# ubisoft/ubisoft-laforge-msmd

Hardware: AMD Instinct MI355X
Metric: FLAME frames/sec on 4s@16kHz clips (whole job; MSMD.forward motion-coefficient frames) (higher is better)
Workload: dtype bf16; 1 GPU; configs[1]: MSMD.forward, batch=32 x 4 s clips per GPU, wav2vec2-base encoder + 8-layer motion decoder, eval-mode, synthetic closed-form weights; batch_per_gpu=32, frames_per_clip=100, parallelism=dp1 (independent clips, no collective), launch=one hipGraph replay per step (the batch sits in the captured input buffers)

## Files before the change

### include/msmd_hip.h

```cpp
#ifndef MSMD_HIP_H
#define MSMD_HIP_H

#include <stdint.h>

#ifdef __cplusplus
extern "C" {
#endif

#define MSMD_F32 0
#define MSMD_BF16 1
#define MSMD_F16 2
#define MSMD_F16X2 3

#define MSMD_ACT_NONE 0
#define MSMD_ACT_GELU 1
#define MSMD_ACT_ELU 2

typedef void* msmd_stream_t;

int msmd_abi_version(void);
#define MSMD_GEMM_VARIANT(v) ((v) << 8)
#define MSMD_GEMM_WRITE_THROUGH (1 << 16)
#define MSMD_GEMM_PAIRED_STORES (1 << 17)
#define MSMD_GEMM_STAGGER (1 << 18)
#define MSMD_GEMM_ONE_TILE_PER_WORKGROUP (1 << 19)
#define MSMD_GEMM_NO_256_TILE (1 << 20)
#define MSMD_GEMM_W_BELOW_32 (1 << 21)

int msmd_spin_us(float us, long* ticks_out, msmd_stream_t stream);

int msmd_gemm(const void* A, const void* W, const float* bias, const void* residual, void* C,
              int M, int N, int K, int in_dtype, int out_dtype,
              long lda, int rows_per_batch, long a_batch_stride, long ldw, long ldc, long ldr, int act,
              int batch, long strideA, long strideW, long strideC, long strideBias, long strideR,
              msmd_stream_t stream);

int msmd_gemm_ln(const void* A, const void* W, const float* bias, const void* residual, void* C, int M, int N, int K,
                 int in_dtype, int out_dtype, long lda, long ldw, long ldc, long ldr, int act, const float* a_stats,
                 const float* w_colsum, const float* r_stats, const float* r_gamma, const float* r_beta,
                 float* stats_out, int slab_in, int slab_out, float eps, msmd_stream_t stream);

int msmd_gemm_ex(const void* A, const void* W, const float* bias, const void* residual, void* C, int M, int N, int K,
                 int in_dtype, int out_dtype, long lda, int rows_per_batch, long a_batch_stride, long ldw, long ldc,
                 long ldr, int act, int batch, long strideA, long strideW, long strideC, long strideBias, long strideR,
                 void* z_out, float p_drop, const unsigned long* rng_state, unsigned int site, msmd_stream_t stream);

int msmd_gemm_route(const void* A, const void* W, const float* bias, const void* residual, void* C, int M, int N, int K,
                    int in_dtype, int out_dtype, long lda, int rows_per_batch, long a_batch_stride, long ldw, long ldc,
                    long ldr, int act, int batch, long strideA, long strideW, long strideC, long strideBias, long strideR,
                    void* z_out, float p_drop, const unsigned long* rng_state, unsigned int site, msmd_stream_t stream);
int msmd_gemm_ln_route(const void* A, const void* W, const float* bias, const void* residual, void* C, int M, int N, int K,
                       int in_dtype, int out_dtype, long lda, long ldw, long ldc, long ldr, int act, const float* a_stats,
                       const float* w_colsum, const float* r_stats, const float* r_gamma, const float* r_beta,
                       float* stats_out, int slab_in, int slab_out, float eps, msmd_stream_t stream);

int msmd_gemm_actbwd(const void* A, const void* W, const void* Z, void* C, int M, int N, int K, int in_dtype, int out_dtype,
                     long lda, long ldw, int act, float p_drop, const unsigned long* rng_state, unsigned int site,
                     msmd_stream_t stream);

int msmd_gemm_batched2(const void* A, const void* W, void* C, int M, int N, int K, int in_dtype, int out_dtype,
                       long lda, long ldw, long ldc, int batch_outer, long strideA_o, long strideW_o, long strideC_o,
                       int batch_inner, long strideA_i, long strideW_i, long strideC_i, msmd_stream_t stream);

int msmd_gemm_tn(const void* A, const void* B, float* C, float* colsum, int M, int N, int K, long lda, long ldb,
                 long ldc, int batch, long strideA, long strideB, long strideC, int b_rows_per_window,
                 long b_window_stride, int accumulate, void* ws, long ws_bytes, msmd_stream_t stream);
long msmd_gemm_tn_workspace(int M, int N, int K, int batch);

int msmd_layernorm(const void* x, const void* residual, const float* gamma, const float* beta,
                   const float* post_add, void* y, int rows, int cols, float eps, int act,
                   int in_dtype, int out_dtype, msmd_stream_t stream);
int msmd_layernorm_pre(const void* x, const float* pre_gamma, const float* pre_beta, const void* residual,
                       const float* gamma, const float* beta, void* y, int rows, int cols, float eps, int dtype,
                       msmd_stream_t stream);

int msmd_layernorm_f16x2(const float* x, const float* residual, const float* gamma, const float* beta,
                         const float* post_add, float* y, void* y_split, int rows, int cols, float eps, int act,
                         msmd_stream_t stream);

int msmd_split_f16x2(const float* x, void* y, long rows, int cols, long ldx, int cols_out, msmd_stream_t stream);
int msmd_unsplit_f16x2(const void* x, float* y, long rows, int cols, int cols_in, long ldy, msmd_stream_t stream);

int msmd_attention_prefetch(const void* Q, const void* K, const void* V, void* O, int B, int H, int Tq, int Tk,
                            long q_bstride, long q_tstride, long k_bstride, long k_tstride, long v_bstride,
                            long v_tstride, long o_bstride, long o_tstride, float scale, const uint8_t* mask, int dtype,
                            const void* const* prefetch_ptrs, const long* prefetch_bytes, int n_prefetch,
                            msmd_stream_t stream);
int msmd_attention(const void* Q, const void* K, const void* V, void* O, int B, int H, int Tq, int Tk,
                   long q_bstride, long q_tstride, long k_bstride, long k_tstride, long v_bstride,
                   long v_tstride, long o_bstride, long o_tstride, float scale, const uint8_t* mask,
                   int dtype, msmd_stream_t stream);

int msmd_attention_f16x2(const void* Q, const void* K, const void* V, void* O, int B, int H, int Tq, int Tk,
                         long q_bstride, long q_tstride, long k_bstride, long k_tstride, long v_bstride,
                         long v_tstride, long o_bstride, long o_tstride, float scale, const uint8_t* mask,
                         int out_dtype, msmd_stream_t stream);


int msmd_person_query_attention(const void* x, long x_seq_stride, const void* Wq, const float* bq, const void* K,
                                const void* V, long kv_bstride, long kv_tstride, void* out, int N, int H, int Tk, int d,
                                float scale, int dtype, msmd_stream_t stream);
int msmd_person_query_attention_ln(const void* x, long x_seq_stride, const void* Wq, const float* bq,
                                   const float* wq_colsum, float ln_eps, const void* K, const void* V, long kv_bstride,
                                   long kv_tstride, void* out, int N, int H, int Tk, int d, float scale, int dtype,
                                   msmd_stream_t stream);

int msmd_attention_dropout(const void* Q, const void* K, const void* V, void* O, int B, int H, int Tq, int Tk,
                           long q_bstride, long q_tstride, long k_bstride, long k_tstride, long v_bstride,
                           long v_tstride, long o_bstride, long o_tstride, float scale, const uint8_t* mask,
                           float p_drop, const unsigned long* rng_state, unsigned int site, int dtype,
                           msmd_stream_t stream);
int msmd_attention_dropout_prefetch(const void* Q, const void* K, const void* V, void* O, int B, int H, int Tq, int Tk,
                                    long q_bstride, long q_tstride, long k_bstride, long k_tstride, long v_bstride,
                                    long v_tstride, long o_bstride, long o_tstride, float scale, const uint8_t* mask,
                                    float p_drop, const unsigned long* rng_state, unsigned int site, int dtype,
                                    const void* const* prefetch_ptrs, const long* prefetch_bytes, int n_prefetch,
                                    msmd_stream_t stream);

int msmd_dropout(const void* x, const void* residual, void* y, long n, float p, const unsigned long* rng_state,
                 unsigned int site, int dtype, msmd_stream_t stream);

int msmd_attention_bwd(const void* Q, const void* K, const void* V, const void* dO, void* dQ, void* dK, void* dV,
                       int B, int H, int Tq, int Tk, long q_bstride, long q_tstride, long k_bstride,
                       long k_tstride, long v_bstride, long v_tstride, long do_bstride, long do_tstride,
                       long dq_bstride, long dq_tstride, long dk_bstride, long dk_tstride, long dv_bstride,
                       long dv_tstride, float scale, const uint8_t* mask, float p_drop,
                       const unsigned long* rng_state, unsigned int site, msmd_stream_t stream);

int msmd_pad_audio(const float* audio, float* out, int B, int L, int reflect_len, int replicate_len,
                   msmd_stream_t stream);

#define MSMD_CONV0_SPLITS 16
int msmd_conv0_stats(const float* audio, const float* w0, float* stats, float* ws, int B, int L, int reflect_len,
                     int replicate_len, int C, float eps, msmd_stream_t stream);

int msmd_conv0_gn_gelu(const float* audio, const float* w0, const float* stats, const float* gamma,
                       const float* beta, void* out, int B, int L, int reflect_len, int replicate_len,
                       int C, int out_dtype, msmd_stream_t stream);

int msmd_conv0_ln_gelu(const float* audio, const float* w0, const float* bias, const float* gamma, const float* beta,
                       void* out, int B, int L, int reflect_len, int replicate_len, int C, float eps, int out_dtype,
                       msmd_stream_t stream);

int msmd_interp_linear(const void* x, void* y, int B, int T_in, int T_crop, int T_out, int C, int dtype,
                       msmd_stream_t stream);

int msmd_group_pad(const void* x, void* y, int B, int T, int G, int Cg, int Cg_out, int pad, int dtype, int out_dtype,
                   msmd_stream_t stream);

int msmd_pos_conv(const void* x, const void* w, const float* bias, void* y, int B, int T, int G, int Cg, int kpos,
                  int dtype, msmd_stream_t stream);

int msmd_denoiser_pack_input(const float* motion, const float* eps, const float* c0, const float* c1,
                             const float* prev_motion, const float* indicator, void* feats, int N, int L,
                             int Lp, int dm, int Kpad, int motion_batch, int out_dtype, msmd_stream_t stream);

int msmd_denoiser_pack_input_guided(const float* motion, const float* eps, const float* c0, const float* c1,
                                    const float* prev_motion, const float* indicator, const unsigned char* guide_mask,
                                    const float* guide_values, void* feats, int N, int L, int Lp, int dm, int Kpad,
                                    int motion_batch, int out_dtype, msmd_stream_t stream);

int msmd_add_pe_token(void* x, const float* pe, const void* tok0, const void* row0_add, int N, int T, int d,
                      int dtype, msmd_stream_t stream);

int msmd_heads_static_mix(const void* dec, long ld_dec, const void* stat, float* out, int N, int L, int dm,
                          int nb, int stat_batch, int use_head_alpha, int dtype, msmd_stream_t stream);

int msmd_cfg_ddpm_step(float* x, const float* res, const float* z, const float* scales, int n_entries,
                       int B, int L, int Lp, int dm, int mode, int target, float c0, float c1, float sigma,
                       msmd_stream_t stream);

int msmd_sampler_step_select(const void* emb_all, const float* coef_table, int* t_dev, void* emb_row,
                             float* coefs, int d, int dtype, msmd_stream_t stream);
int msmd_cfg_ddpm_step_dev(float* x, const float* res, const float* z, const float* scales, const float* coefs,
                           int n_entries, int B, int L, int Lp, int dm, int mode, int target, msmd_stream_t stream);

int msmd_cfg_solver_step(float* x, const float* res, const float* z, const float* scales, float* d_prev,
                         int n_entries, int B, int L, int Lp, int dm, int mode, float p0, float p1, float ax,
                         float ath, float b1, float sigma, msmd_stream_t stream);
int msmd_cfg_solver_step_dev(float* x, const float* res, const float* z, const float* scales, float* d_prev,
                             const float* coefs, int n_entries, int B, int L, int Lp, int dm, int mode,
                             msmd_stream_t stream);
int msmd_sampler_solver_select(const void* emb_tab, const float* coef_tab, int* i_dev, void* emb_row,
                               float* coefs, int d, int dtype, msmd_stream_t stream);

int msmd_cfg_streams_step(float* x, const float* res, const void* dec, long ld_dec, const void* stat, const float* z,
                          const float* scales, float* d_prev, float* cum_static, float* theta_dyn, float* theta_alpha,
                          int slot, int n_slots, int n_entries, int B, int L, int Lp, int dm, int nb, int stat_batch,
                          int use_head_alpha, int mode, int dtype, float p0, float p1, float ax, float ath, float b1,
                          float sigma, msmd_stream_t stream);
int msmd_cfg_streams_step_dev(float* x, const float* res, const void* dec, long ld_dec, const void* stat, const float* z,
                              const float* scales, float* d_prev, float* cum_static, float* theta_dyn,
                              float* theta_alpha, const float* coefs, const int* step_dev, int n_slots, int n_entries,
                              int B, int L, int Lp, int dm, int nb, int stat_batch, int use_head_alpha, int mode,
                              int dtype, msmd_stream_t stream);

int msmd_lbs_prepare(const float* betas, const float* pose, const float* JS, const int* parents,
                     float* coef, void* coef_hl, float* A, float* joints, void* at_tiles, int B, int NB, int J, int Kp,
                     int pose_is_matrix, msmd_stream_t stream);
int msmd_flame_prepare(const float* shape, const float* expr, const float* pose6, const float* eye, const float* JS,
                       const int* parents, float* coef, float* A, float* joints, void* skin_tiles, int B, int NS, int NE,
                       int ignore_global_rot, int* shape_varies, float* v_template_folded, const float* dirs,
                       const float* v_template, int Vp, msmd_stream_t stream);
int msmd_lbs_skin(const float* coef, const float* A, const float* v_template, const float* dirs,
                  const float* lbs_weights, float* verts, int B, int J, int V, int Vp, int Kp,
                  msmd_stream_t stream);
int msmd_lbs_skin_bf16x3(const void* coef_hl, const float* A, const float* v_template, const void* dirs_hl,
                         const float* lbs_weights, float* verts, int B, int J, int V, int Vp, int Kp,
                         msmd_stream_t stream);

int msmd_lbs_skin_v2(const void* skin_tiles, const float* v_template, const void* dirs_hl, const float* lbs_weights,
                     float* verts, int B, int J, int V, int Vp, int Kp, const int* shape_varies,
                     const float* v_template_folded, msmd_stream_t stream);

int msmd_lbs_skin_v2_f16(const void* skin_tiles, const float* v_template, const void* dirs, const float* lbs_weights,
                         void* verts16, int B, int J, int V, int V_ld, int Vp, int Kp, const int* shape_varies,
                         const float* v_template_folded, int single_plane, msmd_stream_t stream);
int msmd_lbs_tiles_f16(const void* skin_tiles, void* tiles16, int B, msmd_stream_t stream);

int msmd_lbs_skin_v2_train(const void* skin_tiles, const float* v_template, const void* dirs_hl,
                           const float* lbs_weights, float* verts, float* v_posed, int B, int J, int V, int Vp, int Kp,
                           msmd_stream_t stream);
int msmd_lbs_pack(const float* coef, const float* A, void* coef_hl, void* skin_tiles, int B, int Kp, msmd_stream_t stream);
int msmd_lbs_skin_bwd(const float* grad_verts, const float* v_posed, const float* A, const float* lbs_weights,
                      float* dp_planes, float* dA, int B, int J, int V, int Vp, msmd_stream_t stream);

int msmd_landmarks(const float* verts, const int* faces, const int* lmk_faces_idx, long idx_bstride,
                   const float* bary, long bary_bstride, float* out, int B, int V, int L, msmd_stream_t stream);

int msmd_landmarks_bwd(const float* grad_lmk, const int* faces, const int* lmk_faces_idx, long idx_bstride,
                       const float* bary, long bary_bstride, float* grad_verts, int B, int V, int L, int accumulate,
                       msmd_stream_t stream);

int msmd_dynamic_lmk_row(const float* full_pose, const int* neck_chain, int n_chain, int* row, int B, int J,
                         int pose_is_matrix, msmd_stream_t stream);

int msmd_batch_rodrigues(const float* rot_vecs, float* R, int N, msmd_stream_t stream);
int msmd_batch_rodrigues_bwd(const float* rot_vecs, const float* grad_R, float* grad_rot_vecs, int N, msmd_stream_t stream);

#define MSMD_ROT_QUAT_TO_MAT 0
#define MSMD_ROT_MAT_TO_QUAT 1
#define MSMD_ROT_AA_TO_QUAT 2
#define MSMD_ROT_QUAT_TO_AA 3
#define MSMD_ROT_AA_TO_MAT 4
#define MSMD_ROT_MAT_TO_AA 5
#define MSMD_ROT_6D_TO_MAT 6
#define MSMD_ROT_MAT_TO_6D 7
#define MSMD_ROT_AA_TO_6D 8
#define MSMD_ROT_EULER_TO_MAT 9
#define MSMD_ROT_MAT_TO_EULER 10
#define MSMD_ROT_QUAT_STANDARDIZE 11
#define MSMD_ROT_QUAT_INVERT 12
#define MSMD_ROT_QUAT_RAW_MUL 13
#define MSMD_ROT_QUAT_MUL 14
#define MSMD_ROT_QUAT_APPLY 15
int msmd_rotation_convert(int op, const float* in, const float* in2, float* out, long n, int conv,
                          msmd_stream_t stream);
int msmd_rotation_convert_bwd(int op, const float* in, const float* in2, const float* grad_out, float* grad_in,
                              float* grad_in2, long n, int conv, msmd_stream_t stream);

int msmd_masked_seq_loss(const float* gt, const float* pred, const int* end_idx, float* out, double* acc_ws,
                         int N, int T, int C, int c_lo, int c_hi, int order, int prefix, int criterion, int mode,
                         float scale, msmd_stream_t stream);
int msmd_masked_seq_loss_bwd(const float* gt, const float* pred, const int* end_idx, const double* acc_ws,
                             const float* upstream, float* grad_pred, int N, int T, int C, int c_lo, int c_hi, int order,
                             int prefix, int criterion, int mode, float scale, msmd_stream_t stream);
int msmd_kl_loss(const float* mu, const float* logvar, float* out, double* acc_ws, long n, msmd_stream_t stream);
int msmd_truncate_rows(float* x, const int* end_idx, int N, int L, int inner, int unit, int replicate,
                       msmd_stream_t stream);
int msmd_adam_step(float* param, const float* grad, float* exp_avg, float* exp_avg_sq, long n, float lr,
                   float beta1, float beta2, float eps, int step, float grad_scale, msmd_stream_t stream);

int msmd_comm_version(void);
int msmd_comm_unique_id(void* id_out_128_bytes);
int msmd_comm_init(void** comm_out, int world, int rank, const void* id_128_bytes);
int msmd_comm_destroy(void* comm);
int msmd_allreduce_bucket(void* comm, void* buf, long n, int dtype, msmd_stream_t stream);

int msmd_transpose(const void* x, void* y, int rows, int cols, long ldx, long ldy, int batch, long stride_x,
                   long stride_y, int batch_inner, long stride_x_i, long stride_y_i, int dtype, msmd_stream_t stream);
long msmd_colsum_workspace(long rows, int cols);
int msmd_colsum(const void* x, float* out, long rows, int cols, long ld, int accumulate, int dtype, void* ws, long ws_bytes,
                msmd_stream_t stream);
int msmd_act_fwd(const void* z, void* y, long n, int act, int dtype, msmd_stream_t stream);
int msmd_act_bwd(const void* dy, const void* z, void* dz, long n, int act, int dtype, msmd_stream_t stream);
int msmd_act_bwd_dropout(const void* dy, const void* z, void* dz, long n, int act, float p,
                         const unsigned long* rng_state, unsigned int site, int dtype, msmd_stream_t stream);
int msmd_layernorm_bwd(const void* dy, const void* x, const float* gamma, void* dx, float* dgamma, float* dbeta,
                       int rows, int cols, float eps, int dtype, void* ws, long ws_bytes, msmd_stream_t stream);
long msmd_layernorm_bwd_workspace(int rows, int cols);
int msmd_layernorm_bwd_dropout(const void* dy, const void* x, const float* gamma, void* dx, void* dx_drop, float* dgamma,
                               float* dbeta, int rows, int cols, float eps, float p_drop, const unsigned long* rng_state,
                               unsigned int site, int dtype, void* ws, long ws_bytes, msmd_stream_t stream);
int msmd_softmax_rows(void* s, const uint8_t* mask, long rows, int cols, int ld, int Tq, float scale, int dtype,
                      msmd_stream_t stream);
int msmd_softmax_bwd_rows(const void* P, void* dP, long rows, int cols, int ld, float scale, int dtype,
                          msmd_stream_t stream);

int msmd_unfold_t(const void* xp, void* out, int B, int T, int Tp, int G, int Cg, int Kk, long ld_out, int dtype,
                  msmd_stream_t stream);

int msmd_cast(const void* x, void* y, long n, int in_dtype, int out_dtype, msmd_stream_t stream);
int msmd_pad_cols(const void* x, void* y, long rows, int cols_in, int cols_out, int in_dtype, int out_dtype,
                  msmd_stream_t stream);
int msmd_mean_time(const void* x, float* y, int B, int T, int C, int dtype, msmd_stream_t stream);

int msmd_dynamic_threshold(float* res, int N, int T_all, int L, int C, float ratio, float dt_min, float dt_max,
                           msmd_stream_t stream);

int msmd_cast_transpose_multi(const float* base, const long* meta, int n_weights, long total_tiles, void* cast_arena,
                              void* transposed_arena, msmd_stream_t stream);

int msmd_batch_windows(const float* audio_flat, const float* coef_flat, const long* desc, const float* clip_stats,
                       const float* coef_mean, const float* coef_std, float* out_audio, float* out_motion, int B, int L,
                       int C, int n_audio, double audio_unit, msmd_stream_t stream);

int msmd_render_vertices(const float* verts, const int* faces, const int* csr_offsets, const int* csr_faces,
                         const float* view, const float* t_center, const float* rot, float* screen, float* normals,
                         int B, int V, int F, float focal, int H, int W, msmd_stream_t stream);
int msmd_render_raster(const float* screen, const float* normals, const int* faces, const float* shade,
                       const float* lights, int n_lights, void* rgba, float* depth, int* face_id, int B, int V, int F,
                       int H, int W, float near, float far, unsigned background, msmd_stream_t stream);

long msmd_texture_texels(int Ht, int Wt);
int msmd_texture_mips(const void* img, int Ht, int Wt, int channels, float* pyramid, msmd_stream_t stream);
int msmd_render_shade_textured(const float* screen, const float* normals, const int* faces, const float* vt, const int* ft,
                               const float* pyramid, int Ht, int Wt, const float* shade, const float* lights,
                               int n_lights, const int* face_id, void* rgba, float* uvl, int B, int V, int F, int Nt,
                               int H, int W, float near, msmd_stream_t stream);

#define MSMD_TEX_PLANAR_F32 0
#define MSMD_TEX_IMAGE_U8 1
int msmd_flametex_forward(const float* mean, const float* basis, const float* code, void* out, int out_format, int n_copies,
                          int Hs, int Ws, int Hd, int Wd, int n_tex, msmd_stream_t stream);
long msmd_flametex_backward_workspace(int Hd, int Wd, int n_tex);
int msmd_flametex_backward(const float* basis, const float* grad_out, int n_copies, float* grad_code, float* workspace,
                           int Hs, int Ws, int Hd, int Wd, int n_tex, msmd_stream_t stream);

#define MSMD_AUDIO_RUN 256
int msmd_audio_resample(const void* pcm, long pcm_elems, int is_int16, const long* desc, int n_clips, long max_out_len,
                        int L, int M, int taps, const float* bank, float* out, long out_elems, double* partials,
                        msmd_stream_t stream);
int msmd_audio_znorm(float* out, long out_elems, const long* desc, int n_clips, long max_out_len, const double* partials,
                     double* stats, msmd_stream_t stream);

#define MSMD_JPEG_RESTART_INTERVAL 32
#define MSMD_JPEG_MAX_SIDE 16384
int msmd_jpeg_intervals(int H, int W);
int msmd_jpeg_coefficients(const void* frames, long frame_stride, long row_stride, int pixel_stride, int B, int H, int W,
                           int quality, short* coef, msmd_stream_t stream);
int msmd_jpeg_measure(const short* coef, int B, int H, int W, int header_len, int* interval_len, long* interval_rel,
                      long* frame_size, long* offsets, msmd_stream_t stream);
int msmd_jpeg_write(const short* coef, int B, int H, int W, const void* header, int header_len, const long* interval_rel,
                    const long* offsets, void* out, long out_bytes, msmd_stream_t stream);

#ifdef __cplusplus
}
// ... 3 lines not shown
```

### ubisoft-laforge-msmd_amd/csrc/gemm.hip

```cpp
#include "common.h"
#include <atomic>
#include <utility>

struct GemmArgs {
  const void* A; const void* W; const float* bias; const void* R; void* C;
  int M, N, K;
  long lda; int rows_per_batch; long a_batch_stride; long ldw, ldc, ldr;
  int act; int vec_ok; float inv_rpb;
  long strideA, strideW, strideC, strideBias, strideR;
  int mt, nt;
  int batch_inner; long strideA2, strideW2, strideC2;
  void* Z; float p_drop; const unsigned long* rng; unsigned site;
  int xn;
  int flags;
  const float* a_stats = nullptr; int a_nt = 0; const float* w_colsum = nullptr;
  const float* r_stats = nullptr; int r_nt = 0; const float* r_gamma = nullptr; const float* r_beta = nullptr;
  float* stats_out = nullptr; float ln_eps = 1e-5f;
  int stagger_ticks = 0;
};

enum : int {
  GF_WRITE_THROUGH = 1, GF_PAIRED_STORES = 2, GF_STAGGER = 4,
  GF_ACT_BWD = 8,
  GF_ONE_TILE = 16, GF_NO_256 = 32,
  GF_W_BELOW_32 = 64,
};
struct GemmActWord { int act, hint, flags; };
static constexpr GemmActWord gemm_unpack_act(int act) {
  return {act & 0xff, (act >> 8) & 0xff, ((act >> 16) & 7) | (((act >> 19) & 7) << 4)};
}
static_assert(gemm_unpack_act(MSMD_GEMM_WRITE_THROUGH).flags == GF_WRITE_THROUGH && gemm_unpack_act(MSMD_GEMM_PAIRED_STORES).flags == GF_PAIRED_STORES &&
              gemm_unpack_act(MSMD_GEMM_STAGGER).flags == GF_STAGGER && gemm_unpack_act(MSMD_GEMM_ONE_TILE_PER_WORKGROUP).flags == GF_ONE_TILE &&
              gemm_unpack_act(MSMD_GEMM_NO_256_TILE).flags == GF_NO_256 && gemm_unpack_act(MSMD_GEMM_W_BELOW_32).flags == GF_W_BELOW_32 && gemm_unpack_act(~0).flags == (0x7f & ~GF_ACT_BWD),
              "internal flag bits follow include/msmd_hip.h; no bit of `act` sets the internal one");
enum : int {
  GV_GENERIC = 0,
  GV_SPLIT_128 = 1, GV_SPLIT_64 = 5,
  GV_64_DEEP = 9, GV_64 = 12,
  GV_256x64 = 14,
  GV_192 = 15,
  GV_128 = 17,
  GV_128_AB = 13, GV_128_ONE_AB = 66,
  GV_256 = 80,
};

enum GemmEpi : int { EPI_ALL = 0, EPI_PLAIN = 1, EPI_LN_OPERAND = 2, EPI_LN_RESIDUAL = 3 };
constexpr int ACT_RUNTIME = -1;
constexpr int epia(GemmEpi e, int act) { return e + 10 * (1 + act); }
constexpr GemmEpi epia_family(int code) { return (GemmEpi)(code % 10); }
constexpr int epia_act(int code) { return code / 10 - 1; }

template <typename T> struct Mfma;
template <> struct Mfma<bf16_t> {
  static __device__ __forceinline__ void run(const u32x4& a, const u32x4& b, f32x4& acc) {
    acc = __builtin_amdgcn_mfma_f32_16x16x32_bf16(__builtin_bit_cast(bf16x8, a), __builtin_bit_cast(bf16x8, b),
                                                  acc, 0, 0, 0);
  }
};
template <> struct Mfma<f16_t> {
  static __device__ __forceinline__ void run(const u32x4& a, const u32x4& b, f32x4& acc) {
    acc = __builtin_amdgcn_mfma_f32_16x16x32_f16(__builtin_bit_cast(f16x8, a), __builtin_bit_cast(f16x8, b), acc, 0, 0, 0);
  }
};
template <> struct Mfma<float> {
  static __device__ __forceinline__ void run(const u32x4& a, const u32x4& b, f32x4& acc) {
#pragma unroll
    for (int e = 0; e < 4; ++e)
      acc = __builtin_amdgcn_mfma_f32_16x16x4f32(__uint_as_float(a[e]), __uint_as_float(b[e]), acc, 0, 0, 0);
  }
};

__device__ __forceinline__ int lds_off(int row, int chunk) { return row * 128 + ((chunk ^ ((row >> 1) & 7)) << 4); }

__device__ __forceinline__ long a_row_offset(const GemmArgs& p, int m) {
  if (p.rows_per_batch >= p.M) return (long)m * p.lda;
  int q = (int)((float)m * p.inv_rpb);
  int r = m - q * p.rows_per_batch;
  if (r < 0) { q -= 1; r += p.rows_per_batch; }
  if (r >= p.rows_per_batch) { q += 1; r -= p.rows_per_batch; }
  return (long)q * p.a_batch_stride + (long)r * p.lda;
}

template <typename TO> __device__ __forceinline__ float act_out(float x, int act) {
  if (act == MSMD_ACT_GELU) return sizeof(TO) == 2 ? gelu_poly16(x) : gelu_erf(x);
  if (act == MSMD_ACT_ELU) return elu1(x);
  return x;
}
template <typename TO, int ACT> __device__ __forceinline__ float act_out_c(float x, int act) {
  if constexpr (ACT == MSMD_ACT_GELU) return sizeof(TO) == 2 ? gelu_poly16(x) : gelu_erf(x);
  else if constexpr (ACT == MSMD_ACT_ELU) return elu1(x);
  else if constexpr (ACT == MSMD_ACT_NONE) return x;
  else return act_out<TO>(x, act);
}

__device__ __forceinline__ void store16_wt(void* p, const u32x4 v) {
  asm volatile("global_store_dwordx4 %0, %1, off sc1\n\ts_nop 1" ::"v"(p), "v"(v) : "memory");
}
__device__ __forceinline__ void store8_wt(void* p, const u32x2 v) {
  asm volatile("global_store_dwordx2 %0, %1, off sc1\n\ts_nop 1" ::"v"(p), "v"(v) : "memory");
}
template <typename TO> __device__ __forceinline__ void store4_out(TO* p, const float* v, bool wt) {
  if constexpr (sizeof(TO) == 4) {
    const f32x4 o = f32x4{v[0], v[1], v[2], v[3]};
    if (wt) store16_wt(p, __builtin_bit_cast(u32x4, o));
    else *(f32x4*)p = o;
  } else {
    const typename Vec4T<TO>::type o = pack4<TO>(v[0], v[1], v[2], v[3]);
    if (wt) store8_wt(p, __builtin_bit_cast(u32x2, o));
    else *(typename Vec4T<TO>::type*)p = o;
  }
}

template <typename TO, int FM, int FN, bool AB, bool LEAN, int ACT>
__device__ __forceinline__ void gemm_epilogue_interior(const GemmArgs& p, const f32x4 (&acc)[FN][FM], int z, int m_base,
                                                         int n_base, int fr, int fq) {
  TO* __restrict__ C = (TO*)p.C + (z / p.batch_inner) * p.strideC + (z % p.batch_inner) * p.strideC2 +
                       (long)(m_base + fr) * p.ldc + n_base + fq * 4;
  const TO* __restrict__ R = p.R ? (const TO*)p.R + z * p.strideR + (long)(m_base + fr) * p.ldr + n_base + fq * 4 : nullptr;
  const float* __restrict__ bias = p.bias ? p.bias + z * p.strideBias + n_base + fq * 4 : nullptr;
  const bool wt = p.flags & GF_WRITE_THROUGH;
  f32x4 bv[FN];
#pragma unroll
  for (int i = 0; i < FN; ++i) bv[i] = bias ? *(const f32x4*)(bias + i * 16) : f32x4{0.f, 0.f, 0.f, 0.f};
  typedef typename Vec4T<TO>::type V4;
  constexpr int RJ = sizeof(TO) == 2 ? FM : 1;
  V4 rr[RJ][FN];
  auto load_residual = [&](int j0) {
    if (R) {
#pragma unroll
      for (int j = 0; j < RJ; ++j)
#pragma unroll
        for (int i = 0; i < FN; ++i) rr[j][i] = *(const V4*)(R + (long)(j0 + j) * 16 * p.ldr + i * 16);
    }
  };
  if constexpr (RJ == FM) load_residual(0);
  auto finish = [&](int i, int j, float (&v)[4]) {
    TO* crow = C + (long)j * 16 * p.ldc;
#pragma unroll
    for (int e = 0; e < 4; ++e) v[e] = acc[i][j][e] + bv[i][e];
    if (AB && (p.flags & GF_ACT_BWD)) {
      const V4 z4 = *(const V4*)((const TO*)p.Z + (crow + i * 16 - (TO*)p.C));
#pragma unroll
      for (int e = 0; e < 4; ++e) v[e] *= act_grad_fast((float)z4[e], ACT >= 0 ? ACT : p.act);
    } else {
      if (!LEAN && p.Z) store4_out<TO>((TO*)p.Z + (crow + i * 16 - (TO*)p.C), v, wt);
#pragma unroll
      for (int e = 0; e < 4; ++e) v[e] = act_out_c<TO, ACT>(v[e], p.act);
    }
    if (!LEAN && p.p_drop > 0.f) {
      const long idx = (long)(m_base + j * 16 + fr) * p.N + (n_base + i * 16 + fq * 4);
      const Philox4 rb = dropout_bits(p.rng, p.site, (unsigned long)(idx >> 2));
      const unsigned thr = dropout_threshold(p.p_drop);
      const float c = 1.0f / (1.0f - p.p_drop);
      v[0] = rb.x >= thr ? v[0] * c : 0.f;
      v[1] = rb.y >= thr ? v[1] * c : 0.f;
      v[2] = rb.z >= thr ? v[2] * c : 0.f;
      v[3] = rb.w >= thr ? v[3] * c : 0.f;
    }
    if (R) {
#pragma unroll
      for (int e = 0; e < 4; ++e) v[e] += (float)rr[j % RJ][i][e];
    }
  };
  if constexpr (sizeof(TO) == 2 && FM % 2 == 0) {
    if (p.flags & GF_PAIRED_STORES) {
      const bool odd = fq & 1;
#pragma unroll
      for (int jp = 0; jp < FM / 2; ++jp) {
#pragma unroll
        for (int i = 0; i < FN; ++i) {
          float v0[4], v1[4];
          finish(i, 2 * jp, v0);
          finish(i, 2 * jp + 1, v1);
          const u32x2 a = __builtin_bit_cast(u32x2, pack4<TO>(v0[0], v0[1], v0[2], v0[3]));
          const u32x2 b = __builtin_bit_cast(u32x2, pack4<TO>(v1[0], v1[1], v1[2], v1[3]));
          const u32x2 send = odd ? a : b;
          u32x2 recv;
          recv[0] = __shfl_xor(send[0], 16, 64);
          recv[1] = __shfl_xor(send[1], 16, 64);
          const u32x4 o = odd ? u32x4{recv[0], recv[1], b[0], b[1]} : u32x4{a[0], a[1], recv[0], recv[1]};
          TO* dst = C + (long)(2 * jp + (odd ? 1 : 0)) * 16 * p.ldc + i * 16 - (odd ? 4 : 0);
          if (wt) store16_wt(dst, o);
          else *(u32x4*)dst = o;
        }
      }
      return;
    }
  }
#pragma unroll
  for (int j = 0; j < FM; ++j) {
    if constexpr (RJ != FM) load_residual(j);
#pragma unroll
    for (int i = 0; i < FN; ++i) {
      float v[4];
      finish(i, j, v);
      store4_out<TO>(C + (long)j * 16 * p.ldc + i * 16, v, wt);
    }
  }
}

template <typename TO, int FM, int FN, bool AB = false, bool LEAN = false, int ACT = -1>
__device__ __forceinline__ void gemm_epilogue(const GemmArgs& p, const f32x4 (&acc)[FN][FM], int z, int m_base,
                                              int n_base, int fr, int fq) {
  if (p.vec_ok && m_base + FM * 16 <= p.M && n_base + FN * 16 <= p.N) {
    gemm_epilogue_interior<TO, FM, FN, AB, LEAN, ACT>(p, acc, z, m_base, n_base, fr, fq);
    return;
  }
  TO* __restrict__ C = (TO*)p.C + (z / p.batch_inner) * p.strideC + (z % p.batch_inner) * p.strideC2;
  const TO* __restrict__ R = p.R ? (const TO*)p.R + z * p.strideR : nullptr;
  const float* __restrict__ bias = p.bias ? p.bias + z * p.strideBias : nullptr;
#pragma unroll
  for (int i = 0; i < FN; ++i) {
    const int n = n_base + i * 16 + fq * 4;
    if (n >= p.N) continue;
    float bv[4] = {0.f, 0.f, 0.f, 0.f};
    if (bias) {
#pragma unroll
      for (int e = 0; e < 4; ++e) bv[e] = (n + e < p.N) ? bias[n + e] : 0.f;
    }
#pragma unroll
    for (int j = 0; j < FM; ++j) {
      const int m = m_base + j * 16 + fr;
      if (m >= p.M) continue;
      float v[4];
#pragma unroll
      for (int e = 0; e < 4; ++e) v[e] = acc[i][j][e] + bv[e];
      TO* cp = C + (long)m * p.ldc + n;
      if (AB && (p.flags & GF_ACT_BWD)) {
        const TO* zp = (const TO*)p.Z + (cp - (TO*)p.C);
#pragma unroll
        for (int e = 0; e < 4; ++e)
          if (n + e < p.N) v[e] *= act_grad_fast((float)zp[e], ACT >= 0 ? ACT : p.act);
      } else {
        if (!LEAN && p.Z) {
          TO* zp = (TO*)p.Z + (cp - (TO*)p.C);
#pragma unroll
          for (int e = 0; e < 4; ++e)
            if (n + e < p.N) zp[e] = (TO)v[e];
        }
#pragma unroll
        for (int e = 0; e < 4; ++e) v[e] = act_out_c<TO, ACT>(v[e], p.act);
      }
      if (!LEAN && p.p_drop > 0.f) {
        const Philox4 rb = dropout_bits(p.rng, p.site, (unsigned long)(((long)m * p.N + n) >> 2));
        const unsigned thr = dropout_threshold(p.p_drop);
        const float c = 1.0f / (1.0f - p.p_drop);
        v[0] = rb.x >= thr ? v[0] * c : 0.f;
        v[1] = rb.y >= thr ? v[1] * c : 0.f;
        v[2] = rb.z >= thr ? v[2] * c : 0.f;
        v[3] = rb.w >= thr ? v[3] * c : 0.f;
      }
      if (p.vec_ok && n + 3 < p.N) {
        if (R) {
          const TO* rp = R + (long)m * p.ldr + n;
          if constexpr (sizeof(TO) == 4) {
            const f32x4 r = *(const f32x4*)rp;
#pragma unroll
            for (int e = 0; e < 4; ++e) v[e] += r[e];
          } else {
            const typename Vec4T<TO>::type r = *(const typename Vec4T<TO>::type*)rp;
#pragma unroll
            for (int e = 0; e < 4; ++e) v[e] += (float)r[e];
          }
        }
        store4_out<TO>(cp, v, p.flags & GF_WRITE_THROUGH);
      } else {
#pragma unroll
        for (int e = 0; e < 4; ++e) {
          if (n + e < p.N) {
            float o = v[e];
            if (R) o += to_f32(R[(long)m * p.ldr + n + e]);
            cp[e] = from_f32<TO>(o);
          }
        }
      }
    }
  }
}

template <int FM>
__device__ __forceinline__ void ln_issue(const float* stats, int nt, int M, int m_base, int fr, int fq, f32x2 (&raw)[FM][4]) {
#pragma unroll
  for (int j = 0; j < FM; ++j) {
    const f32x2* sp = (const f32x2*)stats + min(m_base + j * 16 + fr, M - 1);
#pragma unroll
    for (int q = 0; q < 4; ++q) raw[j][q] = fq + 4 * q < nt ? sp[(long)(fq + 4 * q) * M] : f32x2{0.f, 0.f};
  }
}

template <int FM>
__device__ __forceinline__ void ln_finish(const float* stats, int nt, int M, int m_base, int fr, int fq, const f32x2 (&raw)[FM][4],
                                          float inv_cols, float eps, float (&mu)[FM], float (&rs)[FM]) {
#pragma unroll
  for (int j = 0; j < FM; ++j) {
    float S = (raw[j][0][0] + raw[j][1][0]) + (raw[j][2][0] + raw[j][3][0]);
    float Q = (raw[j][0][1] + raw[j][1][1]) + (raw[j][2][1] + raw[j][3][1]);
    if (nt > 16) {
      const f32x2* sp = (const f32x2*)stats + min(m_base + j * 16 + fr, M - 1);
      for (int t = 16 + fq; t < nt; t += 4) { const f32x2 w = sp[(long)t * M]; S += w[0]; Q += w[1]; }
    }
    S += __shfl_xor(S, 16, 64); S += __shfl_xor(S, 32, 64);
    Q += __shfl_xor(Q, 16, 64); Q += __shfl_xor(Q, 32, 64);
    mu[j] = S * inv_cols;
    rs[j] = rsqrtf(fmaxf(Q * inv_cols - mu[j] * mu[j], 0.f) + eps);
  }
}

template <typename TO, int FM, int FN, int MODE, int ACT = -1>
__device__ __forceinline__ void gemm_epilogue_ln(const GemmArgs& p, const f32x4 (&acc)[FN][FM], int m_base, int n_base,
                                                 int fr, int fq, const f32x2 (&raw)[FM][4]) {
  static_assert((FN == 4 || FN == 2) && (FM >= 2 && FM <= 4), "one wave = one statistics slab of 16 FN columns, 2 to 4 fragment rows");
  constexpr int SLAB = FN * 16;
  constexpr int IB = FM == 3 ? 2 : FN;
  typedef typename Vec4T<TO>::type V4;
  const int n = n_base + fq * 4;
  float mu[FM], rs[FM];
#pragma unroll
  for (int j = 0; j < FM; ++j) { mu[j] = 0.f; rs[j] = 1.f; }
  if constexpr (MODE == 1) ln_finish<FM>(p.a_stats, p.a_nt, p.M, m_base, fr, fq, raw, 1.0f / (float)p.K, p.ln_eps, mu, rs);
  else if (p.r_stats) ln_finish<FM>(p.r_stats, p.r_nt, p.M, m_base, fr, fq, raw, 1.0f / (float)p.N, p.ln_eps, mu, rs);
  float rowS[FM], rowQ[FM], tS[FM], tQ[FM], prS[FM], prQ[FM];
#pragma unroll
  for (int j = 0; j < FM; ++j) rowS[j] = rowQ[j] = tS[j] = tQ[j] = prS[j] = prQ[j] = 0.f;
  const bool odd = fq & 1;
  const bool pair = sizeof(TO) == 2 && (p.flags & GF_PAIRED_STORES);
#pragma unroll
  for (int i0 = 0; i0 < FN; i0 += IB) {
    f32x4 bv[IB], xv[IB], yv[IB];
    V4 rr[FM][IB];
#pragma unroll
    for (int ii = 0; ii < IB; ++ii) bv[ii] = *(const f32x4*)(p.bias + n + (i0 + ii) * 16);
    if constexpr (MODE == 1) {
#pragma unroll
      for (int ii = 0; ii < IB; ++ii) xv[ii] = *(const f32x4*)(p.w_colsum + n + (i0 + ii) * 16);
    } else {
#pragma unroll
// ... 321 lines not shown
  run_epilogue();
}

template <typename TO, int BM, int BN, int WM, int WN, typename TI, int EPIA>
__global__ __launch_bounds__(WM * WN * 64, 4) void gemm2p_kernel(const GemmArgs p) {
  constexpr int EPI = epia_family(EPIA), ACTK = epia_act(EPIA);
  constexpr int NW = WM * WN, NT = NW * 64;
  constexpr int STAGE = (BM + BN) * 128;
  constexpr int LPT = (BM + BN) * 8 / NT;
  constexpr int FM = BM / WM / 16, FN = BN / WN / 16;
  static_assert(EPI >= 1 && EPI <= 3 && sizeof(TO) == 2 && NW == 8 && WN == 2 && BN == 128 && (FM == 2 || FM == 3), "the hot 8-wave tiles, inference epilogues");
  static_assert((BM + BN) * 8 % NT == 0, "tile chunks must divide over the threads");
  constexpr bool LN_LATE = FM == 3;
  extern __shared__ __attribute__((aligned(16))) unsigned char smem[];
  const int tid = threadIdx.x;
  const int xm_n = 8 / p.xn, ntx = (p.nt + p.xn - 1) / p.xn;
  const int vgrid = ((p.mt + xm_n - 1) / xm_n) * ntx * 8;
  const TI* __restrict__ A = (const TI*)p.A;
  const TI* __restrict__ W = (const TI*)p.W;
  auto next_tile = [&](int vb, int& m0, int& n0) -> int {
    for (; vb < vgrid; vb += gridDim.x) {
      const int xcd = vb & 7, slot = vb >> 3;
      const int m_tile = (slot / ntx) * xm_n + (xcd % xm_n), n_tile = (slot % ntx) * p.xn + xcd / xm_n;
      if (m_tile < p.mt && n_tile < p.nt) { m0 = m_tile * BM; n0 = n_tile * BN; return vb; }
    }
    return -1;
  };
  const TI* src[LPT];
  auto set_src = [&](int m0, int n0, int t) {
    const int lane = t & 63, wid = t >> 6;
#pragma unroll
    for (int i = 0; i < LPT; ++i) {
      const int id = (i * NW + wid) * 64 + lane;
      const int row = id >> 3, phys = id & 7;
      const int c = phys ^ ((row >> 1) & 7);
      if (row < BM) src[i] = A + a_row_offset(p, min(m0 + row, p.M - 1)) + c * 8;
      else src[i] = W + (long)min(n0 + row - BM, p.N - 1) * p.ldw + c * 8;
    }
  };
  auto issue = [&](int kt, int stage, int t) {
    const int wid = t >> 6;
#pragma unroll
    for (int i = 0; i < LPT; ++i)
      __builtin_amdgcn_global_load_lds((gbl_void_t*)(src[i] + kt * 64),
                                       (lds_void_t*)(smem + stage * STAGE + (i * NW + wid) * 1024), 16, 0, 0);
  };
  int m0 = 0, n0 = 0;
  int vb = next_tile(blockIdx.x, m0, n0);
  if (vb < 0) return;
  const int nk = p.K / 64;
  set_src(m0, n0, tid);
  int stage = 0;
  issue(0, 0, tid);
  for (;;) {
    int t_k = tid;
    asm volatile("" : "+v"(t_k));
    const int wm = ((t_k >> 6) / WN) * (BM / WM), wn = ((t_k >> 6) % WN) * (BN / WN);
    const int fr = t_k & 15, fq = (t_k & 63) >> 4;
    f32x2 lnraw[LN_LATE ? 1 : FM][4];
    if constexpr (!LN_LATE && EPI != 1) {
      if constexpr (EPI == 2) ln_issue<FM>(p.a_stats, p.a_nt, p.M, m0 + wm, fr, fq, lnraw);
      else if (p.r_stats) ln_issue<FM>(p.r_stats, p.r_nt, p.M, m0 + wm, fr, fq, lnraw);
    }
    f32x4 acc[FN][FM];
#pragma unroll
    for (int i = 0; i < FN; ++i)
#pragma unroll
      for (int j = 0; j < FM; ++j) acc[i][j] = f32x4{0.f, 0.f, 0.f, 0.f};
    int m0n = 0, n0n = 0, vbn = -1;
    for (int kt = 0; kt < nk; ++kt) {
      asm volatile("s_waitcnt vmcnt(0)" ::: "memory");
      __builtin_amdgcn_s_barrier();
      if (kt + 1 < nk) {
        issue(kt + 1, stage ^ 1, t_k);
      } else {
        vbn = next_tile(vb + (int)gridDim.x, m0n, n0n);
        if (vbn >= 0) { set_src(m0n, n0n, t_k); issue(0, stage ^ 1, t_k); }
      }
      const unsigned char* sa = smem + stage * STAGE;
      const unsigned char* sw = sa + BM * 128;
      u32x4 fx[2][FM], fw[2][FN];
#pragma unroll
      for (int g = 0; g < 2; ++g) {
#pragma unroll
        for (int j = 0; j < FM; ++j) fx[g][j] = *(const u32x4*)(sa + lds_off(wm + j * 16 + fr, g * 4 + fq));
#pragma unroll
        for (int i = 0; i < FN; ++i) fw[g][i] = *(const u32x4*)(sw + lds_off(wn + i * 16 + fr, g * 4 + fq));
      }
      __builtin_amdgcn_sched_barrier(0);
#pragma unroll
      for (int g = 0; g < 2; ++g) {
#pragma unroll
        for (int i = 0; i < FN; ++i)
#pragma unroll
          for (int j = 0; j < FM; ++j) Mfma<TI>::run(fw[g][i], fx[g][j], acc[i][j]);
        __builtin_amdgcn_sched_barrier(0);
      }
      stage ^= 1;
    }
    int t_e = tid;
    asm volatile("" : "+v"(t_e));
    const int wm_e = ((t_e >> 6) / WN) * (BM / WM), wn_e = ((t_e >> 6) % WN) * (BN / WN);
    const int fr_e = t_e & 15, fq_e = (t_e & 63) >> 4;
    if constexpr (EPI == 1) {
      gemm_epilogue<TO, FM, FN, false, true, ACTK>(p, acc, 0, m0 + wm_e, n0 + wn_e, fr_e, fq_e);
    } else if constexpr (!LN_LATE) {
      gemm_epilogue_ln<TO, FM, FN, EPI - 1, ACTK>(p, acc, m0 + wm_e, n0 + wn_e, fr_e, fq_e, lnraw);
    } else {
      f32x2 late[FM][4];
      if constexpr (EPI == 2) ln_issue<FM>(p.a_stats, p.a_nt, p.M, m0 + wm_e, fr_e, fq_e, late);
      else if (p.r_stats) ln_issue<FM>(p.r_stats, p.r_nt, p.M, m0 + wm_e, fr_e, fq_e, late);
      gemm_epilogue_ln<TO, FM, FN, EPI - 1, ACTK>(p, acc, m0 + wm_e, n0 + wn_e, fr_e, fq_e, late);
    }
    if (vbn < 0) break;
    vb = vbn; m0 = m0n; n0 = n0n;
    asm volatile("" : "+s"(m0), "+s"(n0));
    int t_s = tid;
    asm volatile("" : "+v"(t_s));
    set_src(m0, n0, t_s);
  }
}

template <int ACT> __device__ __forceinline__ float act_split(float x, int act) {
  if constexpr (ACT == MSMD_ACT_GELU) return gelu_fast(x);
  else if constexpr (ACT == MSMD_ACT_NONE) return x;
  else return act == MSMD_ACT_GELU ? gelu_fast(x) : apply_act(x, act);
}

template <int FM, int FN, int ACT = -1>
__device__ __forceinline__ void gemm_epilogue_split(const GemmArgs& p, const f32x4 (&acc)[FN][FM], int z, int m_base,
                                                    int n_base, int fr, int fq) {
  f16_t* __restrict__ C = (f16_t*)p.C + 2 * ((z / p.batch_inner) * p.strideC + (z % p.batch_inner) * p.strideC2);
  const f16_t* __restrict__ R = p.R ? (const f16_t*)p.R + 2 * (z * p.strideR) : nullptr;
  const float* __restrict__ bias = p.bias ? p.bias + z * p.strideBias : nullptr;
  if (m_base + FM * 16 <= p.M && n_base + FN * 16 <= p.N) {
    const int n = n_base + fq * 4;
    f32x4 bv[FN];
#pragma unroll
    for (int i = 0; i < FN; ++i) bv[i] = bias ? *(const f32x4*)(bias + n + i * 16) : f32x4{0.f, 0.f, 0.f, 0.f};
    f16x4 rh[FM][FN], rl[FM][FN];
    if (R) {
#pragma unroll
      for (int j = 0; j < FM; ++j) {
        const f16_t* rrow = R + (long)(m_base + j * 16 + fr) * 2 * p.ldr;
#pragma unroll
        for (int i = 0; i < FN; ++i) {
          const f16_t* q = rrow + split_col(n + i * 16);
          rh[j][i] = *(const f16x4*)q;
          rl[j][i] = *(const f16x4*)(q + 32);
        }
      }
    }
#pragma unroll
    for (int j = 0; j < FM; ++j) {
      f16_t* crow = C + (long)(m_base + j * 16 + fr) * 2 * p.ldc;
#pragma unroll
      for (int i = 0; i < FN; ++i) {
        float v[4];
#pragma unroll
        for (int e = 0; e < 4; ++e) v[e] = act_split<ACT>(acc[i][j][e] + bv[i][e], p.act);
        if (R) {
#pragma unroll
          for (int e = 0; e < 4; ++e) v[e] += unsplit_f16x2(rh[j][i][e], rl[j][i][e]);
        }
        store4_split(crow, n + i * 16, v);
      }
    }
    return;
  }
#pragma unroll
  for (int i = 0; i < FN; ++i) {
    const int n = n_base + i * 16 + fq * 4;
    if (n >= p.N) continue;
    const f32x4 bv = bias ? *(const f32x4*)(bias + n) : f32x4{0.f, 0.f, 0.f, 0.f};
#pragma unroll
    for (int j = 0; j < FM; ++j) {
      const int m = m_base + j * 16 + fr;
      if (m >= p.M) continue;
      float v[4];
#pragma unroll
      for (int e = 0; e < 4; ++e) v[e] = act_split<ACT>(acc[i][j][e] + bv[e], p.act);
      if (R) {
        float r[4];
        load4_split(R + (long)m * 2 * p.ldr, n, r);
#pragma unroll
        for (int e = 0; e < 4; ++e) v[e] += r[e];
      }
      store4_split(C + (long)m * 2 * p.ldc, n, v);
    }
  }
}

template <typename TO, int BM, int BN, int WM, int WN, int NSTAGE, int ACTK = -1, bool WS = false>
__global__ __launch_bounds__(WM * WN * 64) void gemm2s_kernel(const GemmArgs p) {
  constexpr int NW = WM * WN, NT = NW * 64;
  constexpr int STAGE = (BM + BN) * 128;
  constexpr int LPT = (BM + BN) * 8 / NT;
  constexpr int FM = BM / WM / 16, FN = BN / WN / 16;
  static_assert((BM + BN) * 8 % NT == 0, "tile chunks must divide over the threads");
  extern __shared__ __attribute__((aligned(16))) unsigned char smem[];

  const int pid = blockIdx.x;
  const int xcd = pid & 7, slot = pid >> 3;
  const int xm_n = 8 / p.xn, ntx = (p.nt + p.xn - 1) / p.xn;
  const int m_tile = (slot / ntx) * xm_n + (xcd % xm_n), n_tile = (slot % ntx) * p.xn + xcd / xm_n;
  if (m_tile >= p.mt || n_tile >= p.nt) return;
  const int z = blockIdx.z;
  const int zo = z / p.batch_inner, zi = z % p.batch_inner;
  const f16_t* __restrict__ A = (const f16_t*)p.A + zo * p.strideA + zi * p.strideA2;
  const f16_t* __restrict__ W = (const f16_t*)p.W + zo * p.strideW + zi * p.strideW2;
  const int m0 = m_tile * BM, n0 = n_tile * BN;
  const int tid = threadIdx.x, lane = tid & 63, wid = tid >> 6;

  const f16_t* src[LPT];
#pragma unroll
  for (int i = 0; i < LPT; ++i) {
    const int id = (i * NW + wid) * 64 + lane;
    const int row = id >> 3, phys = id & 7;
    const int c = phys ^ ((row >> 1) & 7);
    if (row < BM) src[i] = A + a_row_offset(p, min(m0 + row, p.M - 1)) + c * 8;
    else src[i] = W + (long)min(n0 + row - BM, p.N - 1) * p.ldw + c * 8;
  }
  auto issue = [&](int kt, int stage) {
#pragma unroll
    for (int i = 0; i < LPT; ++i)
      __builtin_amdgcn_global_load_lds((gbl_void_t*)(src[i] + kt * 64),
                                       (lds_void_t*)(smem + stage * STAGE + (i * NW + wid) * 1024), 16, 0, 0);
  };

  const int wm = (wid / WN) * (BM / WM), wn = (wid % WN) * (BN / WN);
  const int fr = lane & 15, fq = lane >> 4;
  f32x4 acc0[FN][FM], acc1[FN][FM];
#pragma unroll
  for (int i = 0; i < FN; ++i)
#pragma unroll
    for (int j = 0; j < FM; ++j) acc0[i][j] = acc1[i][j] = f32x4{0.f, 0.f, 0.f, 0.f};

  const int nk = p.K / 32;
#pragma unroll
  for (int s = 0; s < NSTAGE - 1; ++s)
    if (s < nk) issue(s, s);
  int stage = 0;
  for (int kt = 0; kt < nk; ++kt) {
    if (kt + NSTAGE - 2 < nk) asm volatile("s_waitcnt vmcnt(%0)" ::"n"((NSTAGE - 2) * LPT) : "memory");
    else asm volatile("s_waitcnt vmcnt(0)" ::: "memory");
    __builtin_amdgcn_s_barrier();
    if (kt + NSTAGE - 1 < nk) issue(kt + NSTAGE - 1, (stage + NSTAGE - 1) % NSTAGE);
    const unsigned char* sa = smem + stage * STAGE;
    const unsigned char* sw = sa + BM * 128;
    u32x4 ah[FM], al[FM], wh[FN], wl[FN];
#pragma unroll
    for (int j = 0; j < FM; ++j) {
      ah[j] = *(const u32x4*)(sa + lds_off(wm + j * 16 + fr, fq));
      al[j] = *(const u32x4*)(sa + lds_off(wm + j * 16 + fr, 4 + fq));
    }
#pragma unroll
    for (int i = 0; i < FN; ++i) {
      wh[i] = *(const u32x4*)(sw + lds_off(wn + i * 16 + fr, fq));
      wl[i] = *(const u32x4*)(sw + lds_off(wn + i * 16 + fr, 4 + fq));
    }
    if constexpr (WS) {
      u32x4 ws[FN];
#pragma unroll
      for (int i = 0; i < FN; ++i) {
        f16x8 h = __builtin_bit_cast(f16x8, wh[i]);
        h = h * (f16_t)MSMD_SPLIT_SCALE;
        ws[i] = __builtin_bit_cast(u32x4, h);
      }
#pragma unroll
      for (int i = 0; i < FN; ++i)
#pragma unroll
        for (int j = 0; j < FM; ++j) Mfma<f16_t>::run(wh[i], al[j], acc0[i][j]);
#pragma unroll
      for (int i = 0; i < FN; ++i)
#pragma unroll
        for (int j = 0; j < FM; ++j) Mfma<f16_t>::run(wl[i], ah[j], acc0[i][j]);
#pragma unroll
      for (int i = 0; i < FN; ++i)
#pragma unroll
        for (int j = 0; j < FM; ++j) Mfma<f16_t>::run(ws[i], ah[j], acc0[i][j]);
    } else {
#pragma unroll
      for (int i = 0; i < FN; ++i)
#pragma unroll
        for (int j = 0; j < FM; ++j) {
          Mfma<f16_t>::run(wh[i], ah[j], acc0[i][j]);
          Mfma<f16_t>::run(wh[i], al[j], acc1[i][j]);
          Mfma<f16_t>::run(wl[i], ah[j], acc1[i][j]);
        }
    }
    stage = (stage + 1 == NSTAGE) ? 0 : stage + 1;
  }
#pragma unroll
  for (int i = 0; i < FN; ++i)
#pragma unroll
    for (int j = 0; j < FM; ++j)
#pragma unroll
      for (int e = 0; e < 4; ++e)
        acc0[i][j][e] = WS ? acc0[i][j][e] * MSMD_SPLIT_INV : fmaf(acc1[i][j][e], MSMD_SPLIT_INV, acc0[i][j][e]);
  if constexpr (sizeof(TO) == 4) gemm_epilogue<float, FM, FN, false, false, ACTK>(p, acc0, z, m0 + wm, n0 + wn, fr, fq);
  else gemm_epilogue_split<FM, FN, ACTK>(p, acc0, z, m0 + wm, n0 + wn, fr, fq);
}

template <typename TI, int EPIA, int SPLIT = 0>
__global__ __launch_bounds__(512) __attribute__((amdgpu_waves_per_eu(2, 2))) void gemm8_kernel(const GemmArgs p) {
  typedef typename std::conditional<(SPLIT & 3) == 2, float, TI>::type TO;
  constexpr bool WS = (SPLIT & 4) != 0;
  constexpr int EPI = epia_family(EPIA), ACTK = epia_act(EPIA);
  static_assert(SPLIT == 0 || (EPI == 1 && __is_same(TI, f16_t)), "split operands: fp16 planes, plain epilogue");
  constexpr int HALF = 128 * 128;
  constexpr int BUF = 4 * HALF;
  extern __shared__ __attribute__((aligned(16))) unsigned char smem[];

  const int pid = blockIdx.x, ntiles = p.mt * p.nt, nwg = gridDim.x;
  const int xcd = pid & 7;
  const int run0 = (xcd < (ntiles & 7) ? xcd * ((ntiles >> 3) + 1) : (ntiles & 7) * ((ntiles >> 3) + 1) + (xcd - (ntiles & 7)) * (ntiles >> 3));
  const int run_n = (ntiles >> 3) + (xcd < (ntiles & 7) ? 1 : 0);
  const int stride = (nwg >> 3) + (xcd < (nwg & 7) ? 1 : 0);
  int tl = pid >> 3;
  const bf16_t* __restrict__ A = (const bf16_t*)p.A;
  const bf16_t* __restrict__ W = (const bf16_t*)p.W;
  const int tid = threadIdx.x, lane = tid & 63;
  const int wid = __builtin_amdgcn_readfirstlane(tid >> 6);
  const int wr = wid >> 2, wc = wid & 3;

  unsigned src[4][2];
  int m0 = 0, n0 = 0;
  auto set_tile = [&](int t) {
    const int m_tile = (run0 + t) / p.nt, n_tile = (run0 + t) - m_tile * p.nt;
    m0 = m_tile * 256; n0 = n_tile * 256;
    int ln = lane;
    asm volatile("" : "+v"(ln));
#pragma unroll
    for (int i = 0; i < 2; ++i) {
      const int row = (i * 8 + wid) * 8 + (ln >> 3), phys = ln & 7;
      const int c = phys ^ ((row >> 1) & 7);
#pragma unroll
      for (int h = 0; h < 2; ++h) {
        src[h][i] = (unsigned)((a_row_offset(p, min(m0 + h * 128 + row, p.M - 1)) + c * 8) * 2);
        src[2 + h][i] = (unsigned)(((long)min(n0 + h * 128 + row, p.N - 1) * p.ldw + c * 8) * 2);
      }
    }
  };
  const unsigned dma_base = wid * 1024;
  auto stage = [&](int which, int kt, unsigned bufoff) {
#pragma unroll
    for (int i = 0; i < 2; ++i)
      __builtin_amdgcn_global_load_lds((gbl_void_t*)((const char*)(which < 2 ? A : W) + (size_t)(src[which][i] + (unsigned)kt * 128u)),
                                       (lds_void_t*)(smem + (dma_base + bufoff + which * HALF + i * 8192)), 16, 0, 0);
  };

  const int fr = lane & 15, fq = lane >> 4;
  const int sw = (fr >> 1) & 7;
  const unsigned ch0 = (fq ^ sw) << 4;
  unsigned xa0 = (wr * 64 + fr) * 128 + ch0, xa1 = xa0 ^ 64;
  unsigned wa0 = 2 * HALF + (wc * 32 + fr) * 128 + ch0, wa1 = wa0 ^ 64;

  f32x4 acc[2][2][2][4];
  u32x4 fx[2][4], fw0[2][2], fw1[2][2];
  u32x4 fs0[2], fs1[2];
  auto scale_w = [&](const u32x4 (&fw)[2][2], u32x4 (&fs)[2]) {
#pragma unroll
    for (int i = 0; i < 2; ++i) {
      f16x8 h = __builtin_bit_cast(f16x8, fw[0][i]);
      h = h * (f16_t)MSMD_SPLIT_SCALE;
      fs[i] = __builtin_bit_cast(u32x4, h);
    }
  };

  auto read_x = [&](int h) {
#pragma unroll
    for (int j = 0; j < 4; ++j) {
      fx[0][j] = *(const u32x4*)(smem + xa0 + h * HALF + j * 2048);
      fx[1][j] = *(const u32x4*)(smem + xa1 + h * HALF + j * 2048);
    }
  };
  auto read_w = [&](int g, u32x4 (&fw)[2][2]) {
#pragma unroll
    for (int i = 0; i < 2; ++i) {
      fw[0][i] = *(const u32x4*)(smem + wa0 + g * HALF + i * 2048);
      fw[1][i] = *(const u32x4*)(smem + wa1 + g * HALF + i * 2048);
    }
  };
  auto quadrant = [&](f32x4 (&a)[2][4], const u32x4 (&fw)[2][2], const u32x4 (&fs)[2]) {
    __builtin_amdgcn_s_setprio(1);
    if constexpr (SPLIT == 0) {
#pragma unroll
      for (int ks = 0; ks < 2; ++ks)
#pragma unroll
        for (int i = 0; i < 2; ++i)
#pragma unroll
          for (int j = 0; j < 4; ++j) Mfma<TI>::run(fw[ks][i], fx[ks][j], a[i][j]);
    } else if constexpr (WS) {
#pragma unroll
      for (int i = 0; i < 2; ++i)
#pragma unroll
        for (int j = 0; j < 4; ++j) Mfma<TI>::run(fw[0][i], fx[1][j], a[i][j]);
#pragma unroll
      for (int i = 0; i < 2; ++i)
#pragma unroll
        for (int j = 0; j < 4; ++j) Mfma<TI>::run(fw[1][i], fx[0][j], a[i][j]);
#pragma unroll
      for (int i = 0; i < 2; ++i)
#pragma unroll
        for (int j = 0; j < 4; ++j) Mfma<TI>::run(fs[i], fx[0][j], a[i][j]);
    } else {
      f32x4 t[2][4];
#pragma unroll
      for (int i = 0; i < 2; ++i)
#pragma unroll
        for (int j = 0; j < 4; ++j) { t[i][j] = f32x4{0.f, 0.f, 0.f, 0.f}; Mfma<TI>::run(fw[0][i], fx[1][j], t[i][j]); }
#pragma unroll
      for (int i = 0; i < 2; ++i)
#pragma unroll
        for (int j = 0; j < 4; ++j) Mfma<TI>::run(fw[1][i], fx[0][j], t[i][j]);
#pragma unroll
      for (int i = 0; i < 2; ++i)
#pragma unroll
        for (int j = 0; j < 4; ++j) {
#pragma unroll
          for (int e = 0; e < 4; ++e) a[i][j][e] = fmaf(t[i][j][e], MSMD_SPLIT_INV, a[i][j][e]);
          Mfma<TI>::run(fw[0][i], fx[0][j], a[i][j]);
        }
      __builtin_amdgcn_sched_group_barrier(0x008, 11, 0);
#pragma unroll
      for (int q = 0; q < 8; ++q) {
        __builtin_amdgcn_sched_group_barrier(0x002, 4, 0);
        __builtin_amdgcn_sched_group_barrier(0x008, 1, 0);
      }
      __builtin_amdgcn_sched_group_barrier(0x008, 5, 0);
    }
    __builtin_amdgcn_s_setprio(0);
  };
#define G8_BAR()                        \
  do {                                  \
    __builtin_amdgcn_sched_barrier(0);  \
    __builtin_amdgcn_s_barrier();       \
    __builtin_amdgcn_sched_barrier(0);  \
  } while (0)
#define G8_EBAR()                                      \
  do {                                                 \
    asm volatile("s_waitcnt lgkmcnt(0)" ::: "memory"); \
    __builtin_amdgcn_s_barrier();                      \
  } while (0)

  const float* ln_stats = EPI == 2 ? p.a_stats : p.r_stats;
  const int ln_nt = EPI == 2 ? p.a_nt : p.r_nt;
  auto ln_request = [&]() {
    if constexpr (EPI >= 2) {
      if (ln_stats) {
        int ll = lane;
        asm volatile("" : "+v"(ll));
        const int m = min(m0 + ((ll >> 2) & 3) * 64 + wid * 8 + (ll & 3) * 2, p.M - 2);
#pragma unroll
        for (int q = 0; q < 4; ++q) {
          if (4 * q < ln_nt) {
            const int t = min(4 * q + (ll >> 4), ln_nt - 1);
            __builtin_amdgcn_global_load_lds((gbl_void_t*)(ln_stats + ((long)t * p.M + m) * 2),
                                             (lds_void_t*)(smem + (2 * BUF + wid * 4096 + q * 1024)), 16, 0, 0);
          }
        }
      }
    }
  };

  const int nk = p.K / (SPLIT ? 32 : 64);
  typedef typename Vec4T<TO>::type V4;
  const bool has_r = p.R != nullptr;
  const bool wt = p.flags & GF_WRITE_THROUGH;

  set_tile(tl);
  ln_request();
  stage(2, 0, 0); stage(0, 0, 0); stage(3, 0, 0); stage(1, 0, 0);
  stage(2, 1, BUF); stage(0, 1, BUF); stage(3, 1, BUF);
  asm volatile("s_waitcnt vmcnt(6)" ::: "memory");
  __builtin_amdgcn_s_barrier();

  while (true) {
    if (wr == 1) __builtin_amdgcn_s_barrier();
#pragma unroll
    for (int h = 0; h < 2; ++h)
#pragma unroll
      for (int g = 0; g < 2; ++g)
#pragma unroll
        for (int i = 0; i < 2; ++i)
#pragma unroll
          for (int j = 0; j < 4; ++j) acc[h][g][i][j] = f32x4{0.f, 0.f, 0.f, 0.f};
    unsigned cur = 0;
    auto ktile = [&](int t, auto MODE_) {
      constexpr int MODE = decltype(MODE_)::value;
      read_w(0, fw0);
      __builtin_amdgcn_sched_barrier(0);
      read_x(0);
      if (MODE <= 1) stage(1, t + 1, cur ^ BUF);
      asm volatile("s_waitcnt lgkmcnt(8)" ::: "memory");
      if constexpr (WS) scale_w(fw0, fs0);
      G8_BAR();
      quadrant(acc[0][0], fw0, fs0);
      G8_BAR();
      read_w(1, fw1);
      if (MODE == 0) stage(2, t + 2, cur);
      if constexpr (WS) {
        asm volatile("s_waitcnt lgkmcnt(0)" ::: "memory");
        scale_w(fw1, fs1);
      }
      G8_BAR();
      quadrant(acc[0][1], fw1, fs1);
      G8_BAR();
      read_x(1);
      if (MODE == 0) stage(0, t + 2, cur);
      G8_BAR();
      quadrant(acc[1][1], fw1, fs1);
      G8_BAR();
      if (MODE == 0) stage(3, t + 2, cur);
      if (MODE == 0) asm volatile("s_waitcnt vmcnt(6)" ::: "memory");
      if (MODE == 1) asm volatile("s_waitcnt vmcnt(0)" ::: "memory");
      G8_BAR();
      quadrant(acc[1][0], fw0, fs0);
      G8_BAR();
      cur ^= BUF; xa0 ^= BUF; xa1 ^= BUF; wa0 ^= BUF; wa1 ^= BUF;
    };
    for (int t = 0; t < nk - 2; ++t) ktile(t, std::integral_constant<int, 0>{});
    ktile(nk - 2, std::integral_constant<int, 1>{});
    ktile(nk - 1, std::integral_constant<int, 2>{});
    if (wr == 0) __builtin_amdgcn_s_barrier();
    if (nk & 1) { xa0 ^= BUF; xa1 ^= BUF; wa0 ^= BUF; wa1 ^= BUF; }

    const int em0 = m0, en0 = n0;
    int el = lane;
    asm volatile("" : "+v"(el));
    const int efr = el & 15, efq = el >> 4;
    const int ncol = en0 + el * 4;
    f32x4 cbias = f32x4{0.f, 0.f, 0.f, 0.f}, cx = f32x4{1.f, 1.f, 1.f, 1.f}, cy = f32x4{0.f, 0.f, 0.f, 0.f};
    if (p.bias) cbias = *(const f32x4*)(p.bias + ncol);
    if constexpr (EPI == 2) cx = *(const f32x4*)(p.w_colsum + ncol);
    if constexpr (EPI == 3) {
      if (p.r_stats) { cx = *(const f32x4*)(p.r_gamma + ncol); cy = *(const f32x4*)(p.r_beta + ncol); }
    }
    float mu_l = 0.f, rs_l = 1.f;
    if constexpr (EPI >= 2) {
      if (ln_stats) {
        const int r32 = el & 31;
        const unsigned base = 2 * BUF + wid * 4096 + (((r32 >> 3) * 4 + ((r32 & 7) >> 1)) << 4) + ((r32 & 1) << 3);
        float Sf[4], Qf[4];
#pragma unroll
        for (int f = 0; f < 4; ++f) {
          f32x2 w[4];
#pragma unroll
          for (int q = 0; q < 4; ++q) {
            const int t = f + 4 * q;
            w[q] = *(const f32x2*)(smem + base + (t >> 2) * 1024 + ((t & 3) << 8));
            if (t >= ln_nt) w[q] = f32x2{0.f, 0.f};
          }
          Sf[f] = (w[0][0] + w[1][0]) + (w[2][0] + w[3][0]);
          Qf[f] = (w[0][1] + w[1][1]) + (w[2][1] + w[3][1]);
        }
        if (ln_nt > 16) {
          const f32x2* rp = (const f32x2*)ln_stats + min(em0 + (r32 >> 3) * 64 + wid * 8 + (r32 & 7), p.M - 1);
#pragma unroll
          for (int f = 0; f < 4; ++f)
            for (int t = 16 + f; t < ln_nt; t += 4) { const f32x2 w = rp[(long)t * p.M]; Sf[f] += w[0]; Qf[f] += w[1]; }
        }
        const float S = (Sf[0] + Sf[1]) + (Sf[2] + Sf[3]), Q = (Qf[0] + Qf[1]) + (Qf[2] + Qf[3]);
        const float inv_cols = 1.0f / (float)(EPI == 2 ? p.K : p.N);
        mu_l = S * inv_cols;
        rs_l = rsqrtf(fmaxf(Q * inv_cols - mu_l * mu_l, 0.f) + p.ln_eps);
        asm volatile("s_waitcnt lgkmcnt(0)" ::: "memory");
      }
    }
    tl += stride;
    const bool more = tl < run_n;
    if (more) {
      set_tile(tl);
      stage(2, 0, 0); stage(0, 0, 0); stage(3, 0, 0); stage(1, 0, 0);
      ln_request();
    }
    auto write_block = [&](const f32x4 (&q0)[2][4], const f32x4 (&q1)[2][4]) {
#pragma unroll
      for (int g = 0; g < 2; ++g)
#pragma unroll
        for (int i = 0; i < 2; ++i)
#pragma unroll
          for (int j = 0; j < 4; ++j) {
            const int row = j * 16 + efr, c = g * 32 + wc * 8 + i * 4 + efq;
            *(f32x4*)(smem + BUF + row * 1024 + ((c ^ efr) << 4)) = g == 0 ? q0[i][j] : q1[i][j];
          }
    };
    auto finish_block = [&](int ps) {
      if constexpr ((SPLIT & 3) == 2) {
        f32x4 rr[8];
        if (has_r) {
#pragma unroll
          for (int it = 0; it < 8; ++it) {
            const int m = min(em0 + ps * 64 + wid * 8 + it, p.M - 1);
            rr[it] = *(const f32x4*)((const float*)p.R + (long)m * p.ldr + ncol);
          }
        }
#pragma unroll
        for (int it = 0; it < 8; ++it) {
          const int row = wid * 8 + it, m = em0 + ps * 64 + row;
          const f32x4 a = *(const f32x4*)(smem + BUF + row * 1024 + ((el ^ (row & 15)) << 4));
          f32x4 o;
#pragma unroll
          for (int e = 0; e < 4; ++e) {
            o[e] = act_out_c<float, ACTK>(WS ? fmaf(a[e], MSMD_SPLIT_INV, cbias[e]) : a[e] + cbias[e], p.act);
            if (has_r) o[e] += rr[it][e];
          }
          if (m < p.M) {
            if (wt) store16_wt((float*)p.C + (long)m * p.ldc + ncol, __builtin_bit_cast(u32x4, o));
            else *(f32x4*)((float*)p.C + (long)m * p.ldc + ncol) = o;
          }
        }
      } else if constexpr ((SPLIT & 3) == 1) {
        const bool odd = el & 1;
        const long coff = 2L * en0 + ((el >> 3) << 6) + (((el >> 1) & 3) << 3) + (odd ? 32 : 0);
        auto swap1 = [](unsigned x) { return (unsigned)__builtin_amdgcn_mov_dpp((int)x, 0xB1, 0xF, 0xF, false); };
        u32x4 rr[8];
        if (has_r) {
#pragma unroll
          for (int it = 0; it < 8; ++it) {
            const int m = min(em0 + ps * 64 + wid * 8 + it, p.M - 1);
            rr[it] = *(const u32x4*)((const f16_t*)p.R + (long)m * 2 * p.ldr + coff);
          }
        }
#pragma unroll
        for (int it = 0; it < 8; ++it) {
          const int row = wid * 8 + it, m = em0 + ps * 64 + row;
          const f32x4 a = *(const f32x4*)(smem + BUF + row * 1024 + ((el ^ (row & 15)) << 4));
          float v[4];
#pragma unroll
          for (int e = 0; e < 4; ++e) v[e] = act_split<ACTK>(WS ? fmaf(a[e], MSMD_SPLIT_INV, cbias[e]) : a[e] + cbias[e], p.act);
          if (has_r) {
            const unsigned g0 = swap1(odd ? rr[it][0] : rr[it][2]), g1 = swap1(odd ? rr[it][1] : rr[it][3]);
            const f16x2 h01 = __builtin_bit_cast(f16x2, odd ? g0 : rr[it][0]), h23 = __builtin_bit_cast(f16x2, odd ? g1 : rr[it][1]);
            const f16x2 l01 = __builtin_bit_cast(f16x2, odd ? rr[it][2] : g0), l23 = __builtin_bit_cast(f16x2, odd ? rr[it][3] : g1);
            v[0] += unsplit_f16x2(h01[0], l01[0]); v[1] += unsplit_f16x2(h01[1], l01[1]);
            v[2] += unsplit_f16x2(h23[0], l23[0]); v[3] += unsplit_f16x2(h23[1], l23[1]);
          }
          f16_t h[4], l[4];
#pragma unroll
          for (int e = 0; e < 4; ++e) split_f16x2(v[e], h[e], l[e]);
          const unsigned hp0 = __builtin_bit_cast(unsigned, f16x2{h[0], h[1]}), hp1 = __builtin_bit_cast(unsigned, f16x2{h[2], h[3]});
          const unsigned lp0 = __builtin_bit_cast(unsigned, f16x2{l[0], l[1]}), lp1 = __builtin_bit_cast(unsigned, f16x2{l[2], l[3]});
          const unsigned g0 = swap1(odd ? hp0 : lp0), g1 = swap1(odd ? hp1 : lp1);
          const u32x4 o = odd ? u32x4{g0, g1, lp0, lp1} : u32x4{hp0, hp1, g0, g1};
          if (m < p.M) {
            if (wt) store16_wt((f16_t*)p.C + (long)m * 2 * p.ldc + coff, o);
            else *(u32x4*)((f16_t*)p.C + (long)m * 2 * p.ldc + coff) = o;
          }
        }
      } else {
      V4 rr[8];
      if (EPI != 2 && has_r) {
#pragma unroll
        for (int it = 0; it < 8; ++it) {
          const int m = min(em0 + ps * 64 + wid * 8 + it, p.M - 1);
          rr[it] = *(const V4*)((const TO*)p.R + (long)m * p.ldr + ncol);
        }
      }
#pragma unroll
      for (int it = 0; it < 8; ++it) {
        const int row = wid * 8 + it, m = em0 + ps * 64 + row;
        const f32x4 a = *(const f32x4*)(smem + BUF + row * 1024 + ((el ^ (row & 15)) << 4));
        float mu = 0.f, rs = 1.f;
        if constexpr (EPI >= 2) {
          mu = __int_as_float(__builtin_amdgcn_readlane(__float_as_int(mu_l), ps * 8 + it));
          rs = __int_as_float(__builtin_amdgcn_readlane(__float_as_int(rs_l), ps * 8 + it));
        }
        float v[4];
#pragma unroll
        for (int e = 0; e < 4; ++e) {
          float x = a[e];
          if constexpr (EPI == 2) x = rs * (x - mu * cx[e]);
          v[e] = act_out_c<TO, ACTK>(x + cbias[e], p.act);
          if constexpr (EPI == 3) v[e] += fmaf(((float)rr[it][e] - mu) * rs, cx[e], cy[e]);
          else if (has_r) v[e] += (float)rr[it][e];
        }
        const V4 o = pack4<TO>(v[0], v[1], v[2], v[3]);
        if (m < p.M) {
          if (wt) store8_wt((TO*)p.C + (long)m * p.ldc + ncol, __builtin_bit_cast(u32x2, o));
          else *(V4*)((TO*)p.C + (long)m * p.ldc + ncol) = o;
        }
        if constexpr (EPI == 3) {
          if (p.stats_out) {
            float S = 0.f, Q = 0.f;
#pragma unroll
            for (int e = 0; e < 4; ++e) { const float w = (float)o[e]; S += w; Q = fmaf(w, w, Q); }
#pragma unroll
            for (int d : {4, 8, 1, 2}) { S += __shfl_xor(S, d, 64); Q += __shfl_xor(Q, d, 64); }
            if ((el & 15) == 0 && m < p.M) *(f32x2*)(p.stats_out + ((long)((en0 >> 6) + (el >> 4)) * p.M + m) * 2) = f32x2{S, Q};
          }
        }
      }
      }
    };
    if (wr == 0) write_block(acc[0][0], acc[0][1]);
    G8_EBAR();
    finish_block(0);
    G8_EBAR();
    if (wr == 1) write_block(acc[0][0], acc[0][1]);
    G8_EBAR();
    finish_block(1);
    G8_EBAR();
    if (wr == 0) write_block(acc[1][0], acc[1][1]);
    G8_EBAR();
    finish_block(2);
    G8_EBAR();
    if (wr == 1) write_block(acc[1][0], acc[1][1]);
    G8_EBAR();
    finish_block(3);
    if (!more) break;
    G8_EBAR();
    set_tile(tl);
    stage(2, 1, BUF); stage(0, 1, BUF); stage(3, 1, BUF);
    asm volatile("s_waitcnt vmcnt(6)" ::: "memory");
    __builtin_amdgcn_s_barrier();
  }
#undef G8_BAR
#undef G8_EBAR
}

template <int... CODES, typename F>
static int dispatch_code(int code, F&& f) {
  int r = -1;
  (void)((code == CODES && ((r = f(std::integral_constant<int, CODES>{})), true)) || ...);
  return r;
}

template <auto KFN>
static int gemm_launch_kernel(dim3 grid, int threads, int lds, hipStream_t st, const GemmArgs& p) {
  if (lds > 0) {
    static std::atomic<unsigned long> allowed{0};
    int dev = 0;
    (void)hipGetDevice(&dev);
    const unsigned long bit = (unsigned)dev < 64 ? 1UL << dev : 0;
    if (!(allowed.load(std::memory_order_relaxed) & bit)) {
      (void)hipFuncSetAttribute((const void*)KFN, hipFuncAttributeMaxDynamicSharedMemorySize, lds);
      allowed.fetch_or(bit, std::memory_order_relaxed);
    }
  }
  hipLaunchKernelGGL(KFN, grid, dim3(threads), lds, st, p);
  MSMD_RETURN_LAST();
}

static int gemm2_xcd_grid(GemmArgs& p, int BM, int BN, long lda) {
  p.mt = (p.M + BM - 1) / BM; p.nt = (p.N + BN - 1) / BN;
  const double a_bytes = 2.0 * p.M * (double)(p.rows_per_batch < p.M ? lda : p.K), w_bytes = 2.0 * p.N * (double)p.K;
  double best = 1e30;
  int want_xn = 1;
  for (int xn = 1; xn <= 4; xn *= 2) {
    const double c = 0.7 * xn * a_bytes + (8.0 / xn) * w_bytes;
    if (c < best && p.nt >= xn) { best = c; want_xn = xn; }
  }
  p.xn = p.nt >= want_xn ? want_xn : 1;
  const int xm_n = 8 / p.xn;
  return ((p.mt + xm_n - 1) / xm_n) * ((p.nt + p.xn - 1) / p.xn) * 8;
}

template <typename TO, int BM, int BN, int WM, int WN, int NSTAGE, bool PIPE = false, typename TI = bf16_t, int EPIA = 0>
static int launch_gemm2(GemmArgs& p, int wgs, int batch, hipStream_t st) {
  constexpr int lds = NSTAGE * (BM + BN) * 128;
  p.stagger_ticks = ((p.flags & GF_STAGGER) && batch == 1 && lds <= 80 * 1024 && (long)p.mt * p.nt > 640)
                        ? (int)(100.0 * 0.5 * ((p.K / 64) * 0.5 + 3.0)) : 0;
  return gemm_launch_kernel<gemm2_kernel<TO, BM, BN, WM, WN, NSTAGE, PIPE, TI, EPIA>>(dim3(wgs, 1, batch), WM * WN * 64, lds, st, p);
}

static int gemm_epia(const GemmArgs& p, bool lnk) {
  GemmEpi e = EPI_ALL;
  if (lnk && p.a_stats) e = EPI_LN_OPERAND;
  else if (lnk && (p.r_stats || p.stats_out)) e = EPI_LN_RESIDUAL;
  else if (!p.a_stats && !p.r_stats && !p.stats_out && !p.Z && !(p.p_drop > 0.f) && !(p.flags & GF_ACT_BWD)) e = EPI_PLAIN;
  return epia(e, p.act == MSMD_ACT_NONE ? MSMD_ACT_NONE : (p.act == MSMD_ACT_GELU && e != EPI_LN_RESIDUAL) ? MSMD_ACT_GELU : ACT_RUNTIME);
}

template <typename TO, int BM, int BN, int WM, int WN, int NSTAGE, bool PIPE = false, typename TI = bf16_t>
static int launch_gemm2_epi(GemmArgs& p, int batch, hipStream_t st) {
  constexpr bool LNK = (BN == 128 || BN == 64) && WN == 2 && (BM / WM / 16 == 2 || BM / WM / 16 == 3) && sizeof(TO) == 2;
  const int code = gemm_epia(p, LNK), wgs = gemm2_xcd_grid(p, BM, BN, p.lda);
  int r;
  if constexpr (LNK && PIPE && NSTAGE == 2 && WM * WN == 8 && BN == 128 && BM == 128) {
    if (batch == 1 && wgs > 512 && !(p.flags & GF_ONE_TILE)) {
      auto persistent = [&](auto c) { return gemm_launch_kernel<gemm2p_kernel<TO, BM, BN, WM, WN, TI, decltype(c)::value>>(dim3(512), WM * WN * 64, 2 * (BM + BN) * 128, st, p); };
      if ((r = dispatch_code<11, 21, 12, 22>(code, persistent)) >= 0) return r;
    }
  }
  auto run = [&](auto c) { return launch_gemm2<TO, BM, BN, WM, WN, NSTAGE, PIPE, TI, decltype(c)::value>(p, wgs, batch, st); };
  if constexpr (LNK) {
    if ((r = dispatch_code<2, 12, 22, 3, 13>(code, run)) >= 0) return r;
  }
  if ((r = dispatch_code<1, 11, 21>(code, run)) >= 0) return r;
  if constexpr (__is_same(TI, bf16_t)) {
    if ((r = dispatch_code<10, 20>(code, run)) >= 0) return r;
  }
  return run(std::integral_constant<int, 0>{});
}

static int gemm8_workgroup_cap() {
  int dev = 0, n = 0;
  if (hipGetDevice(&dev) != hipSuccess || hipDeviceGetAttribute(&n, hipDeviceAttributeMultiprocessorCount, dev) != hipSuccess || n <= 0) n = 256;
  return n;
}

static long gemm_last_row_offset(const GemmArgs& p) {
  return p.rows_per_batch < p.M ? ((long)((p.M - 1) / p.rows_per_batch) * p.a_batch_stride + (long)(p.rows_per_batch - 1) * p.lda) : (long)(p.M - 1) * p.lda;
}

static bool gemm8_takes(const GemmArgs& p, int batch, int osz) {
  if (osz != 2 || batch != 1 || p.batch_inner != 1 || (p.N % 256) || (p.K % 64) || p.K < 128 || !p.vec_ok) return false;
  if (p.Z || p.p_drop > 0.f || (p.flags & GF_ACT_BWD)) return false;
  if (((uintptr_t)p.bias & 15) || ((uintptr_t)p.C & 7) || ((uintptr_t)p.R & 7)) return false;
  if ((gemm_last_row_offset(p) + p.K) * 2 >= (1L << 32) || ((long)(p.N - 1) * p.ldw + p.K) * 2 >= (1L << 32)) return false;
  const GemmEpi epi = epia_family(gemm_epia(p, true));
  if ((p.a_stats || p.r_stats) && ((p.M & 1) || ((uintptr_t)p.a_stats & 15) || ((uintptr_t)p.r_stats & 15))) return false;
  if (epi == EPI_LN_OPERAND && (p.R || !p.bias || !p.w_colsum)) return false;
  if (epi == EPI_LN_RESIDUAL && (!p.R || !p.bias || p.act != MSMD_ACT_NONE)) return false;
  return p.act == MSMD_ACT_NONE || p.act == MSMD_ACT_GELU;
}

static bool gemm8_wins(int M, int N, int K) {
  const long tiles = (long)((M + 255) / 256) * (N / 256);
  if (tiles < 192) return false;
  const double fill = (double)tiles / (256.0 * (double)((tiles + 255) / 256));
  return fill >= 0.75 && (K >= 1024 || fill >= 0.878);
}

constexpr int GEMM8_RING = 2 * 4 * 128 * 128;
template <auto KFN, int LDS>
static int launch_gemm8(GemmArgs& p, hipStream_t st) {
  p.mt = (p.M + 255) / 256; p.nt = p.N / 256;
  const int tiles = p.mt * p.nt, cap = gemm8_workgroup_cap();
  if (tiles <= 512) p.flags |= GF_WRITE_THROUGH;
  return gemm_launch_kernel<KFN>(dim3(tiles < cap ? tiles : cap), 512, LDS, st, p);
}

static bool gemm8s_takes(const GemmArgs& p, int batch, bool split_out) {
  if (batch != 1 || p.batch_inner != 1 || (p.N % 256) || (p.K % 32) || p.K < 64 || !p.vec_ok) return false;
  if (((uintptr_t)p.bias & 15) || ((uintptr_t)p.C & 15) || ((uintptr_t)p.R & 15)) return false;
  if (split_out ? ((p.ldc % 32) || (p.R && (p.ldr % 32))) : ((p.ldc % 4) || (p.R && (p.ldr % 4)))) return false;
  if ((gemm_last_row_offset(p) + 2L * p.K) * 2 >= (1L << 32) || ((long)(p.N - 1) * p.ldw + 2L * p.K) * 2 >= (1L << 32)) return false;
  return p.act == MSMD_ACT_NONE || p.act == MSMD_ACT_GELU;
}
static bool gemm8s_wins(int M, int N, int K, bool w_below_32) {
  const long tiles = (long)((M + 255) / 256) * (N / 256);
  if (tiles < 160) return false;
  const double fill = (double)tiles / (256.0 * (double)((tiles + 255) / 256));
  return fill >= (w_below_32 ? 0.65 : 0.75);
}

template <typename TO, int BM, int BN, int WM, int WN, int NSTAGE>
static int launch_gemm2s(GemmArgs& p, int batch, hipStream_t st) {
  constexpr int lds = NSTAGE * (BM + BN) * 128;
  const dim3 grid(gemm2_xcd_grid(p, BM, BN, p.lda / 2), 1, batch);
  return dispatch_code<0, 1>((p.flags & GF_W_BELOW_32) != 0, [&](auto ws) {
    auto run = [&](auto act) {
      return gemm_launch_kernel<gemm2s_kernel<TO, BM, BN, WM, WN, NSTAGE, decltype(act)::value, decltype(ws)::value != 0>>(grid, WM * WN * 64, lds, st, p);
    };
    int r = -1;
    if constexpr (lds <= 80 * 1024) r = dispatch_code<MSMD_ACT_NONE, MSMD_ACT_GELU>(p.act, run);
    return r >= 0 ? r : run(std::integral_constant<int, ACT_RUNTIME>{});
  });
}

template <typename TO>
static int dispatch_gemm2s(GemmArgs& p, int batch, hipStream_t st, int variant) {
  switch (variant) {
    case GV_SPLIT_128: return launch_gemm2s<TO, 128, 128, 4, 2, 2>(p, batch, st);
    case GV_SPLIT_64: return launch_gemm2s<TO, 64, 64, 2, 2, 4>(p, batch, st);
    case GV_256x64: return launch_gemm2s<TO, 256, 64, 8, 1, 2>(p, batch, st);
    case GV_256:
      if (!gemm8s_takes(p, batch, sizeof(TO) == 2)) return -1;
      return dispatch_code<11, 21>(epia(EPI_PLAIN, p.act), [&](auto c) {
        return dispatch_code<0, 1>((p.flags & GF_W_BELOW_32) != 0, [&](auto ws) {
          return launch_gemm8<gemm8_kernel<f16_t, decltype(c)::value, (sizeof(TO) == 4 ? 2 : 1) + 4 * decltype(ws)::value>, GEMM8_RING>(p, st);
        });
      });
    default: return -1;
  }
}

template <typename T, typename TO>
static int launch_gemm(GemmArgs& p, int batch, hipStream_t st) {
  const bool small = (p.N <= 64) || ((long)((p.M + 127) / 128) * ((p.N + 127) / 128) * batch < 128);
  const int B = small ? 64 : 128;
  p.mt = (p.M + B - 1) / B; p.nt = (p.N + B - 1) / B;
  const dim3 grid(((p.mt + 7) / 8) * 8 * p.nt, 1, batch);
  return small ? gemm_launch_kernel<gemm_kernel<T, TO, 64, 64>>(grid, 256, 0, st, p)
               : gemm_launch_kernel<gemm_kernel<T, TO, 128, 128>>(grid, 256, 0, st, p);
}

static constexpr bool gemm2_has(int variant, bool bf16) {
  if (variant == GV_128_AB || variant == GV_128_ONE_AB) return bf16;
  return variant == GV_64_DEEP || variant == GV_64 || variant == GV_256x64 || variant == GV_192 || variant == GV_128 || variant == GV_256;
}

template <typename TO, typename TI>
static int dispatch_gemm(GemmArgs& p, int batch, hipStream_t st, int variant) {
  if (variant == GV_GENERIC) return launch_gemm<TI, TO>(p, batch, st);
  if constexpr (sizeof(TI) == 2) {
    if (!gemm2_has(variant, __is_same(TI, bf16_t))) return -1;
    if constexpr (__is_same(TI, bf16_t)) {
      if (variant == GV_128_AB) return launch_gemm2<TO, 128, 128, 4, 2, 2>(p, gemm2_xcd_grid(p, 128, 128, p.lda), batch, st);
      if (variant == GV_128_ONE_AB) return launch_gemm2<TO, 128, 128, 4, 2, 2, true>(p, gemm2_xcd_grid(p, 128, 128, p.lda), batch, st);
    }
    switch (variant) {
      case GV_64_DEEP: return launch_gemm2_epi<TO, 64, 64, 2, 2, 4, false, TI>(p, batch, st);
      case GV_64: return launch_gemm2_epi<TO, 64, 64, 2, 2, 2, false, TI>(p, batch, st);
      case GV_256x64: return launch_gemm2_epi<TO, 256, 64, 8, 1, 2, true, TI>(p, batch, st);
      case GV_192: return launch_gemm2_epi<TO, 192, 128, 4, 2, 2, true, TI>(p, batch, st);
      case GV_128: return launch_gemm2_epi<TO, 128, 128, 4, 2, 2, true, TI>(p, batch, st);
    }
    if constexpr (sizeof(TO) == 2) {
      if (!gemm8_takes(p, batch, 2)) return -1;
      return dispatch_code<11, 21, 12, 22, 13>(gemm_epia(p, true), [&](auto c) {
        constexpr int E = decltype(c)::value;
        return launch_gemm8<gemm8_kernel<TI, E>, GEMM8_RING + (epia_family(E) >= EPI_LN_OPERAND ? 8 * 4096 : 0)>(p, st);
      });
    }
  }
  return -1;
}

static bool tall_rounds_favour_192(int M, long tiles128, long tiles192) {
  if (M < 9600 || tiles192 < 256) return false;
  const double fill128 = (double)tiles128 / (512.0 * (double)((tiles128 + 511) / 512));
  const double fill192 = (double)tiles192 / (512.0 * (double)((tiles192 + 511) / 512));
  return 1.2 * fill192 > 1.03 * fill128;
}

struct GemmCall {
  const void* A = nullptr; const void* W = nullptr; const float* bias = nullptr; const void* residual = nullptr; void* C = nullptr;
  int M = 0, N = 0, K = 0, in_dtype = 0, out_dtype = 0;
  long lda = 0; int rows_per_batch = 0; long a_batch_stride = 0; long ldw = 0, ldc = 0, ldr = 0;
  int act = 0;
  int batch = 1; long strideA = 0, strideW = 0, strideC = 0, strideBias = 0, strideR = 0;
  int batch_inner = 1; long strideA2 = 0, strideW2 = 0, strideC2 = 0;
  void* z_out = nullptr; float p_drop = 0.f; const unsigned long* rng = nullptr; unsigned site = 0; int internal_flags = 0;
  const float* a_stats = nullptr; const float* w_colsum = nullptr; const float* r_stats = nullptr; const float* r_gamma = nullptr; const float* r_beta = nullptr;
  float* stats_out = nullptr; int slab_in = 0, slab_out = 0; float eps = 1e-5f;
};

static GemmArgs gemm_args(const GemmCall& c, int act, int flags, int osz, int ab = 1) {
  GemmArgs p{};
  const int rows_per_batch = c.rows_per_batch <= 0 ? c.M : c.rows_per_batch;
  p.A = c.A; p.W = c.W; p.bias = c.bias; p.R = c.residual; p.C = c.C;
  p.M = c.M; p.N = c.N; p.K = c.K;
  p.lda = ab * c.lda; p.rows_per_batch = rows_per_batch; p.a_batch_stride = ab * c.a_batch_stride;
  p.ldw = ab * c.ldw; p.ldc = c.ldc; p.ldr = c.ldr; p.act = act;
  p.inv_rpb = 1.0f / (float)rows_per_batch;
  p.strideA = ab * c.strideA; p.strideW = ab * c.strideW; p.strideC = c.strideC; p.strideBias = c.strideBias; p.strideR = c.strideR;
  p.batch_inner = c.batch_inner; p.strideA2 = ab * c.strideA2; p.strideW2 = ab * c.strideW2; p.strideC2 = c.strideC2;
  p.xn = 1;
  p.vec_ok = osz == 0 ||
             ((c.ldc % 4 == 0) && (c.strideC % 4 == 0) && (c.strideC2 % 4 == 0) && (((uintptr_t)c.C % (4 * osz)) == 0) &&
              (!c.residual || ((c.ldr % 4 == 0) && (c.strideR % 4 == 0) && (((uintptr_t)c.residual % (4 * osz)) == 0))));
  if ((flags & GF_PAIRED_STORES) && (osz != 2 || (c.ldc % 8) || (c.strideC % 8) || (c.strideC2 % 8) || ((uintptr_t)c.C % 16) || !p.vec_ok))
    flags &= ~GF_PAIRED_STORES;
  p.flags = flags;
  return p;
}

static int gemm_split_route(const GemmArgs& p, int nz, bool split_out, int hint, int flags) {
  const bool takes8 = gemm8s_takes(p, nz, split_out);
  if (hint == GV_256 && !takes8) hint = 0;
  if (hint) return (hint == GV_SPLIT_128 || hint == GV_SPLIT_64 || hint == GV_256x64 || hint == GV_256) ? hint : -1;
  if (!(flags & GF_NO_256) && (flags & GF_W_BELOW_32) && takes8 && gemm8s_wins(p.M, p.N, p.K, true)) return GV_256;
  if (p.N <= 64) return (long)((p.M + 255) / 256) * nz >= 256 ? GV_256x64 : GV_SPLIT_64;
  return (long)((p.M + 127) / 128) * ((p.N + 127) / 128) * nz >= 192 ? GV_SPLIT_128 : GV_SPLIT_64;
}

static int gemm16_route(const GemmArgs& p, int nz, int osz, bool bf16, int hint, int flags, int cols = 0) {
  const bool takes8 = (cols != 64 || !p.stats_out) && gemm8_takes(p, nz, osz);
  const bool rule8 = hint == 0 && !(flags & GF_NO_256);
  if (!(hint == GV_256 ? takes8 : !cols || (cols == 128 && (hint == GV_192 || hint == GV_128 || hint == GV_128_ONE_AB)))) hint = 0;
  if (hint) return gemm2_has(hint, bf16) ? hint : GV_GENERIC;
  const int M = p.M, N = p.N;
  const long tiles128 = (long)((M + 127) / 128) * ((N + 127) / 128) * nz;
  const long tiles192 = (long)((M + 191) / 192) * ((N + 127) / 128) * nz;
  const bool wide = cols ? cols == 128 : N > 64;
  if (rule8 && takes8 && gemm8_wins(M, N, p.K)) return GV_256;
  if (wide && M >= 16000 && tiles192 >= 400) return GV_192;
  if (wide && osz == 2 && !p.Z && !(p.p_drop > 0.f) && !(p.flags & GF_ACT_BWD) && tall_rounds_favour_192(M, tiles128, tiles192)) return GV_192;
  if (cols ? wide : wide && tiles128 >= 192) return GV_128;
  if (!cols && N <= 64 && (long)((M + 255) / 256) * nz >= 256) return GV_256x64;
  return p.K >= 1024 ? GV_64_DEEP : GV_64;
}

static int gemm_plan(GemmArgs& p, const GemmCall& c) {
  if (c.M <= 0 || c.N <= 0 || c.K <= 0 || c.batch <= 0 || c.batch_inner <= 0 || !c.A || !c.W || !c.C) return -1;
  const GemmActWord u = gemm_unpack_act(c.act);
  const int flags = u.flags | c.internal_flags, nz = c.batch * c.batch_inner;
  const auto strides_divide = [&](int E) {
    return !(c.K % E || c.lda % E || c.ldw % E || c.a_batch_stride % E || c.strideA % E || c.strideW % E || c.strideA2 % E || c.strideW2 % E);
  };
  if (c.in_dtype == MSMD_F16X2) {
    if (c.out_dtype != MSMD_F32 && c.out_dtype != MSMD_F16X2) return -1;
    if (!strides_divide(32) || c.z_out || c.p_drop != 0.f) return -1;
    if (((uintptr_t)c.A & 15) || ((uintptr_t)c.W & 15) || ((uintptr_t)c.C & 15)) return -1;
    if (c.out_dtype == MSMD_F16X2) {
      if ((c.N & 3) || c.ldc % 32 || c.strideC % 32 || c.strideC2 % 32 || (c.residual && (c.ldr % 32 || c.strideR % 32))) return -1;
      if (c.bias && (((uintptr_t)c.bias & 15) || (c.strideBias & 3))) return -1;
    }
    p = gemm_args(c, u.act, flags & (GF_WRITE_THROUGH | GF_W_BELOW_32), c.out_dtype == MSMD_F32 ? 4 : 0, 2);
    return gemm_split_route(p, nz, c.out_dtype == MSMD_F16X2, u.hint, flags);
  }
  if (c.in_dtype == MSMD_F32 ? (c.out_dtype != MSMD_F32 && c.out_dtype != MSMD_F16 && c.out_dtype != MSMD_BF16)
                             : ((c.in_dtype != MSMD_F16 && c.in_dtype != MSMD_BF16) || (c.out_dtype != c.in_dtype && c.out_dtype != MSMD_F32)))
    return -1;
  if (!strides_divide(c.in_dtype == MSMD_F32 ? 4 : 8)) return -1;
  if (((uintptr_t)c.A & 15) || ((uintptr_t)c.W & 15)) return -1;
  if (c.p_drop != 0.f && (!(c.p_drop > 0.f && c.p_drop < 1.f) || !c.rng || (c.N & 3) || c.ldc != c.N || c.batch != 1 || c.batch_inner != 1))
    return -1;
  const int osz = c.out_dtype == MSMD_F32 ? 4 : 2;
  p = gemm_args(c, u.act, flags, osz);
  p.Z = c.z_out; p.p_drop = c.p_drop; p.rng = c.rng; p.site = c.site;
  if (c.in_dtype == MSMD_F32 || (c.K % 64)) return GV_GENERIC;
  return gemm16_route(p, nz, osz, c.in_dtype == MSMD_BF16, u.hint, flags);
}

static int gemm_launch(GemmArgs& p, int in_dtype, int out_dtype, int nz, int variant, hipStream_t st) {
  switch (in_dtype * 4 + out_dtype) {
    case MSMD_F16X2 * 4 + MSMD_F32: return dispatch_gemm2s<float>(p, nz, st, variant);
    case MSMD_F16X2 * 4 + MSMD_F16X2: return dispatch_gemm2s<f16_t>(p, nz, st, variant);
    case MSMD_BF16 * 4 + MSMD_BF16: return dispatch_gemm<bf16_t, bf16_t>(p, nz, st, variant);
    case MSMD_BF16 * 4 + MSMD_F32: return dispatch_gemm<float, bf16_t>(p, nz, st, variant);
    case MSMD_F16 * 4 + MSMD_F16: return dispatch_gemm<f16_t, f16_t>(p, nz, st, variant);
    case MSMD_F16 * 4 + MSMD_F32: return dispatch_gemm<float, f16_t>(p, nz, st, variant);
    case MSMD_F32 * 4 + MSMD_F32: return dispatch_gemm<float, float>(p, nz, st, variant);
    case MSMD_F32 * 4 + MSMD_F16: return dispatch_gemm<f16_t, float>(p, nz, st, variant);
    case MSMD_F32 * 4 + MSMD_BF16: return dispatch_gemm<bf16_t, float>(p, nz, st, variant);
  }
  return -1;
}

static int gemm_run(int (*plan)(GemmArgs&, const GemmCall&), const GemmCall& c, msmd_stream_t stream) {
  GemmArgs p;
  const int variant = plan(p, c);
  const int r = variant < 0 ? -1 : gemm_launch(p, c.in_dtype, c.out_dtype, c.batch * c.batch_inner, variant, (hipStream_t)stream);
  return r >= 0 ? r : 1;
}

static GemmCall gemm_ex_call(const void* A, const void* W, const float* bias, const void* residual, void* C, int M, int N, int K, int in_dtype,
                             int out_dtype, long lda, int rows_per_batch, long a_batch_stride, long ldw, long ldc, long ldr, int act, int batch,
                             long strideA, long strideW, long strideC, long strideBias, long strideR, void* z_out, float p_drop,
                             const unsigned long* rng_state, unsigned int site) {
  GemmCall c;
  c.A = A; c.W = W; c.bias = bias; c.residual = residual; c.C = C;
  c.M = M; c.N = N; c.K = K; c.in_dtype = in_dtype; c.out_dtype = out_dtype;
  c.lda = lda; c.rows_per_batch = rows_per_batch; c.a_batch_stride = a_batch_stride; c.ldw = ldw; c.ldc = ldc; c.ldr = ldr;
  c.act = act; c.batch = batch;
  c.strideA = strideA; c.strideW = strideW; c.strideC = strideC; c.strideBias = strideBias; c.strideR = strideR;
  c.z_out = z_out; c.p_drop = p_drop; c.rng = rng_state; c.site = site;
  return c;
}

extern "C" int msmd_gemm_ex(const void* A, const void* W, const float* bias, const void* residual, void* C, int M, int N, int K, int in_dtype,
                            int out_dtype, long lda, int rows_per_batch, long a_batch_stride, long ldw, long ldc, long ldr, int act, int batch,
                            long strideA, long strideW, long strideC, long strideBias, long strideR, void* z_out, float p_drop,
                            const unsigned long* rng_state, unsigned int site, msmd_stream_t stream) {
  return gemm_run(gemm_plan, gemm_ex_call(A, W, bias, residual, C, M, N, K, in_dtype, out_dtype, lda, rows_per_batch, a_batch_stride, ldw, ldc, ldr,
                                          act, batch, strideA, strideW, strideC, strideBias, strideR, z_out, p_drop, rng_state, site), stream);
}

extern "C" int msmd_gemm(const void* A, const void* W, const float* bias, const void* residual, void* C, int M, int N, int K, int in_dtype,
                         int out_dtype, long lda, int rows_per_batch, long a_batch_stride, long ldw, long ldc, long ldr, int act, int batch,
                         long strideA, long strideW, long strideC, long strideBias, long strideR, msmd_stream_t stream) {
  return msmd_gemm_ex(A, W, bias, residual, C, M, N, K, in_dtype, out_dtype, lda, rows_per_batch, a_batch_stride, ldw, ldc, ldr,
                      act, batch, strideA, strideW, strideC, strideBias, strideR, nullptr, 0.f, nullptr, 0, stream);
}

extern "C" int msmd_gemm_route(const void* A, const void* W, const float* bias, const void* residual, void* C, int M, int N, int K, int in_dtype,
                               int out_dtype, long lda, int rows_per_batch, long a_batch_stride, long ldw, long ldc, long ldr, int act, int batch,
                               long strideA, long strideW, long strideC, long strideBias, long strideR, void* z_out, float p_drop,
                               const unsigned long* rng_state, unsigned int site, msmd_stream_t) {
  GemmArgs p;
  return gemm_plan(p, gemm_ex_call(A, W, bias, residual, C, M, N, K, in_dtype, out_dtype, lda, rows_per_batch, a_batch_stride, ldw, ldc, ldr,
                                   act, batch, strideA, strideW, strideC, strideBias, strideR, z_out, p_drop, rng_state, site));
}

static int gemm_ln_plan(GemmArgs& p, const GemmCall& c) {
  const int M = c.M, N = c.N, K = c.K;
  if (M <= 0 || N <= 0 || K <= 0 || !c.A || !c.W || !c.C || (K % 64) || (N % 64)) return -1;
  if ((c.in_dtype != MSMD_BF16 && c.in_dtype != MSMD_F16) || c.out_dtype != c.in_dtype) return -1;
  if ((c.lda % 8) || (c.ldw % 8) || (c.ldc % 4) || (c.residual && (c.ldr % 4))) return -1;
  if (((uintptr_t)c.A & 15) || ((uintptr_t)c.W & 15) || ((uintptr_t)c.C & 15) || ((uintptr_t)c.residual & 7) || ((uintptr_t)c.bias & 15)) return -1;
  if ((c.a_stats != nullptr) != (c.w_colsum != nullptr)) return -1;
  if (!c.bias || (c.a_stats && (c.residual || c.stats_out)) || (!c.a_stats && !c.residual)) return -1;
  if (c.r_stats && (!c.residual || !c.r_gamma || !c.r_beta || c.a_stats)) return -1;
  if (((uintptr_t)c.w_colsum & 15) || ((uintptr_t)c.r_gamma & 15) || ((uintptr_t)c.r_beta & 15)) return -1;
  if (((uintptr_t)c.a_stats & 7) || ((uintptr_t)c.r_stats & 7) || ((uintptr_t)c.stats_out & 7)) return -1;
  if ((c.a_stats || c.r_stats) && c.slab_in != 32 && c.slab_in != 64) return -1;
  if (c.stats_out && c.slab_out != 32 && c.slab_out != 64) return -1;
  if ((c.a_stats && (K % c.slab_in)) || (c.r_stats && (N % c.slab_in))) return -1;
  const long tiles128 = (long)((M + 127) / 128) * ((N + 127) / 128);
  const int cols = (c.stats_out ? c.slab_out == 64 : (tiles128 >= 192 && (N % 128) == 0)) ? 128 : 64;
  if (cols == 128 && (N % 128)) return -1;
  const GemmActWord u = gemm_unpack_act(c.act);
  p = gemm_args(c, u.act, GF_PAIRED_STORES | (u.flags & GF_ONE_TILE), 2);
  p.a_stats = c.a_stats; p.a_nt = c.a_stats ? K / c.slab_in : 0; p.w_colsum = c.w_colsum;
  p.r_stats = c.r_stats; p.r_nt = c.r_stats ? N / c.slab_in : 0; p.r_gamma = c.r_gamma; p.r_beta = c.r_beta;
  p.stats_out = c.stats_out; p.ln_eps = c.eps;
  const int variant = gemm16_route(p, 1, 2, c.in_dtype == MSMD_BF16, u.hint, u.flags & GF_NO_256, cols);
  return variant != GV_GENERIC ? variant : -1;
}

static GemmCall gemm_ln_call(const void* A, const void* W, const float* bias, const void* residual, void* C, int M, int N, int K, int in_dtype,
                             int out_dtype, long lda, long ldw, long ldc, long ldr, int act, const float* a_stats, const float* w_colsum,
                             const float* r_stats, const float* r_gamma, const float* r_beta, float* stats_out, int slab_in, int slab_out, float eps) {
  GemmCall c;
  c.A = A; c.W = W; c.bias = bias; c.residual = residual; c.C = C;
  c.M = M; c.N = N; c.K = K; c.in_dtype = in_dtype; c.out_dtype = out_dtype;
  c.lda = lda; c.ldw = ldw; c.ldc = ldc; c.ldr = ldr; c.act = act;
  c.a_stats = a_stats; c.w_colsum = w_colsum; c.r_stats = r_stats; c.r_gamma = r_gamma; c.r_beta = r_beta;
  c.stats_out = stats_out; c.slab_in = slab_in; c.slab_out = slab_out; c.eps = eps;
  return c;
}

extern "C" int msmd_gemm_ln(const void* A, const void* W, const float* bias, const void* residual, void* C, int M, int N, int K, int in_dtype,
                            int out_dtype, long lda, long ldw, long ldc, long ldr, int act, const float* a_stats, const float* w_colsum,
                            const float* r_stats, const float* r_gamma, const float* r_beta, float* stats_out, int slab_in, int slab_out,
                            float eps, msmd_stream_t stream) {
  return gemm_run(gemm_ln_plan, gemm_ln_call(A, W, bias, residual, C, M, N, K, in_dtype, out_dtype, lda, ldw, ldc, ldr, act, a_stats,
                                             w_colsum, r_stats, r_gamma, r_beta, stats_out, slab_in, slab_out, eps), stream);
}

extern "C" int msmd_gemm_ln_route(const void* A, const void* W, const float* bias, const void* residual, void* C, int M, int N, int K,
                                  int in_dtype, int out_dtype, long lda, long ldw, long ldc, long ldr, int act, const float* a_stats,
                                  const float* w_colsum, const float* r_stats, const float* r_gamma, const float* r_beta, float* stats_out,
                                  int slab_in, int slab_out, float eps, msmd_stream_t) {
  GemmArgs p;
  return gemm_ln_plan(p, gemm_ln_call(A, W, bias, residual, C, M, N, K, in_dtype, out_dtype, lda, ldw, ldc, ldr, act, a_stats,
                                      w_colsum, r_stats, r_gamma, r_beta, stats_out, slab_in, slab_out, eps));
}

extern "C" int msmd_gemm_actbwd(const void* A, const void* W, const void* Z, void* C, int M, int N, int K, int in_dtype, int out_dtype, long lda,
                                long ldw, int act, float p_drop, const unsigned long* rng_state, unsigned int site, msmd_stream_t stream) {
  if (!Z || in_dtype != out_dtype || (in_dtype != MSMD_BF16 && in_dtype != MSMD_F16) || (N & 3) || ((uintptr_t)Z & 7)) return 1;
  if (K % 64) return 1;
  GemmCall c;
  c.A = A; c.W = W; c.C = C; c.M = M; c.N = N; c.K = K; c.in_dtype = in_dtype; c.out_dtype = out_dtype;
  c.lda = lda; c.ldw = ldw; c.ldc = N; c.act = act & (0xffff | MSMD_GEMM_WRITE_THROUGH | MSMD_GEMM_PAIRED_STORES);
  c.z_out = const_cast<void*>(Z); c.p_drop = p_drop; c.rng = rng_state; c.site = site; c.internal_flags = GF_ACT_BWD;
  return gemm_run(gemm_plan, c, stream);
}

extern "C" int msmd_gemm_batched2(const void* A, const void* W, void* C, int M, int N, int K, int in_dtype, int out_dtype, long lda, long ldw,
                                  long ldc, int batch_outer, long strideA_o, long strideW_o, long strideC_o, int batch_inner, long strideA_i,
                                  long strideW_i, long strideC_i, msmd_stream_t stream) {
  GemmCall c;
  c.A = A; c.W = W; c.C = C; c.M = M; c.N = N; c.K = K; c.in_dtype = in_dtype; c.out_dtype = out_dtype;
  c.lda = lda; c.ldw = ldw; c.ldc = ldc; c.act = MSMD_ACT_NONE;
  c.batch = batch_outer; c.strideA = strideA_o; c.strideW = strideW_o; c.strideC = strideC_o;
  c.batch_inner = batch_inner; c.strideA2 = strideA_i; c.strideW2 = strideW_i; c.strideC2 = strideC_i;
  return gemm_run(gemm_plan, c, stream);
}
```

### ubisoft-laforge-msmd_amd/ops.py

```python
from __future__ import annotations

import ctypes
import os

import torch
from torch.autograd.function import once_differentiable

from . import _lib

F32, BF16, F16, F16X2 = 0, 1, 2, 3
SPLIT = "f16x2"


class Split:
    __slots__ = ("t", "below_32")
    dtype = SPLIT
    is_cuda = True

    def __init__(self, t, below_32=False):
        if t.dtype != torch.float16 or t.shape[-1] % 64 or t.stride(-1) != 1:
            raise TypeError("Split wraps an fp16 tensor whose last dim is 2 x (a multiple of 32)")
        self.t = t
        self.below_32 = below_32

    @property
    def shape(self):
        return torch.Size((*self.t.shape[:-1], self.t.shape[-1] // 2))

    @property
    def device(self):
        return self.t.device

    def dim(self):
        return self.t.dim()

    def numel(self):
        return self.t.numel() // 2

    def stride(self, i):
        i = i % self.t.dim()
        return 1 if i == self.t.dim() - 1 else self.t.stride(i) // 2

    def data_ptr(self):
        return self.t.data_ptr()

    def is_contiguous(self):
        return self.t.is_contiguous()

    def __getitem__(self, idx):
        if not isinstance(idx, tuple):
            idx = (idx,)
        if Ellipsis in idx:
            k = idx.index(Ellipsis)
            idx = idx[:k] + (slice(None),) * (self.t.dim() - (len(idx) - 1)) + idx[k + 1:]
        if len(idx) == self.t.dim():
            last = idx[-1]
            if not isinstance(last, slice) or last.step not in (None, 1):
                raise IndexError("Split: only contiguous slices along the last dim")
            C = self.shape[-1]
            a, b, _ = last.indices(C)
            if a % 32 or (b % 32 and b != C):
                raise IndexError("Split: last-dim slices must fall on multiples of 32")
            idx = idx[:-1] + (slice(2 * a, 2 * b),)
        return Split(self.t[idx], self.below_32)

    def view(self, *shape):
        shape = shape[0] if len(shape) == 1 and not isinstance(shape[0], int) else shape
        return Split(self.t.view(*shape[:-1], 2 * shape[-1]), self.below_32)

    reshape = view

    def float(self):
        return unsplit(self)


def empty(shape, device, dtype):
    if dtype == SPLIT:
        if shape[-1] % 32:
            raise ValueError("split storage needs a last dim that is a multiple of 32")
        return Split(torch.empty(*shape[:-1], 2 * shape[-1], device=device, dtype=torch.float16))
    return torch.empty(*shape, device=device, dtype=dtype)


def to_split(x, cols_out=None):
    if isinstance(x, Split):
        return x
    _need_cuda(x)
    if x.dtype != torch.float32:
        x = x.float()
    C = x.shape[-1]
    cols_out = (C + 31) // 32 * 32 if cols_out is None else cols_out
    if not x.is_contiguous():
        x = x.contiguous()
    rows = x.numel() // C
    out = torch.empty(*x.shape[:-1], 2 * cols_out, device=x.device, dtype=torch.float16)
    _lib.check(_lib.load().msmd_split_f16x2(_p(x), _p(out), rows, C, C, cols_out, _stream()), "msmd_split_f16x2")
    return Split(out)


def split_weight(w):
    s = to_split(w.float().contiguous())
    s.below_32 = bool(w.numel() == 0 or float(w.detach().abs().max()) < 31.99)
    return s


def unsplit(s, cols=None):
    C = s.shape[-1]
    cols = C if cols is None else cols
    t = s.t if s.t.is_contiguous() else s.t.contiguous()
    rows = t.numel() // (2 * C)
    out = torch.empty(*s.shape[:-1], cols, device=t.device, dtype=torch.float32)
    _lib.check(_lib.load().msmd_unsplit_f16x2(_p(t), _p(out), rows, cols, C, cols, _stream()), "msmd_unsplit_f16x2")
    return out
ACT_NONE, ACT_GELU, ACT_ELU = 0, 1, 2
CONV0_SPLITS = 16

GEMM_TRACE = None
GEMM_FLOPS = None


def _dt(t: torch.Tensor) -> int:
    if t.dtype == SPLIT:
        return F16X2
    if t.dtype == torch.float32:
        return F32
    if t.dtype == torch.bfloat16:
        return BF16
    if t.dtype == torch.float16:
        return F16
    raise TypeError(f"unsupported dtype {t.dtype}")


def _p(t):
    return None if t is None else t.data_ptr()


def _stream():
    return torch.cuda.current_stream().cuda_stream


def _need_cuda(*ts):
    for t in ts:
        if isinstance(t, Split):
            t = t.t
        if t is not None and not t.is_cuda:
            raise RuntimeError("msmd_amd ops need tensors on the MI355X (cuda) device; there is no CPU path")


GEMM_AUTOTUNE = os.environ.get("MSMD_GEMM_AUTOTUNE", "0") == "1"
_TUNE_MIN_FLOP = 1.0e9
_TUNE_CANDIDATES = (17, 13, 9, 12)
_TUNED = {}
GEMM_WRITE_THROUGH, GEMM_PAIRED_STORES, GEMM_STAGGER = 1 << 16, 1 << 17, 1 << 18
GEMM_ONE_TILE_PER_WORKGROUP = 1 << 19
GEMM_NO_256_TILE = 1 << 20
GEMM_W_BELOW_32 = 1 << 21
GEMM_LN_FLAGS = 0
GEMM_LN_ROUTER = None
GEMM_LN_ALL_IN_ONE = False


class capture_guard:

    def __enter__(self):
        import gc
        gc.collect()
        self.was = gc.isenabled()
        gc.disable()
        return self

    def __exit__(self, *exc):
        import gc
        if self.was:
            gc.enable()
        return False
PREFETCH_WEIGHTS = os.environ.get("MSMD_PREFETCH", "1") != "0"
FOLD_LN = os.environ.get("MSMD_FOLD_LN", "1") != "0"
GEMM_ROUTER = None
_GEMM_DEFAULT = {"variant": 0, "flags": GEMM_PAIRED_STORES, "split_variant": 0}
if os.environ.get("MSMD_GEMM_ONE_TILE", "0") == "1":
    _GEMM_DEFAULT["flags"] |= GEMM_ONE_TILE_PER_WORKGROUP
    GEMM_LN_FLAGS = GEMM_ONE_TILE_PER_WORKGROUP


if os.environ.get("MSMD_GEMM_NO_256", "0") == "1":
    _GEMM_DEFAULT["flags"] |= GEMM_NO_256_TILE
    GEMM_LN_FLAGS |= GEMM_NO_256_TILE


class gemm_defaults:

    def __init__(self, variant=None, flags=None, split_variant=None):
        self.new = {k: v for k, v in (("variant", variant), ("flags", flags), ("split_variant", split_variant))
                    if v is not None}

    def __enter__(self):
        self.old = dict(_GEMM_DEFAULT)
        _GEMM_DEFAULT.update(self.new)
        return self

    def __exit__(self, *exc):
        _GEMM_DEFAULT.clear()
        _GEMM_DEFAULT.update(self.old)
        return False


def _trace_begin(M, N, K, batch, dt):
    if GEMM_FLOPS is not None:
        GEMM_FLOPS[0] += 2.0 * M * N * K * batch
    if GEMM_TRACE is None:
        return None
    e0, e1 = torch.cuda.Event(enable_timing=True), torch.cuda.Event(enable_timing=True)
    e0.record()
    return (M, N, K, batch, dt, e0, e1)


def _trace_end(t, route=None, args=None):
    if t is not None:
        t[-1].record()
        GEMM_TRACE.append((*t, route is not None and route(*args) == 80))


def _autotune_gemm(lib, args, key, out, residual):
    if torch.cuda.is_current_stream_capturing() or (residual is not None and residual.data_ptr() == out.data_ptr()):
        return 0
    act = args[16]
    best, best_t = 0, float("inf")
    e0, e1 = torch.cuda.Event(enable_timing=True), torch.cuda.Event(enable_timing=True)
    for v in _TUNE_CANDIDATES:
        args[16] = act | (v << 8)
        if lib.msmd_gemm(*args) != 0:
            continue
        e0.record()
        for _ in range(3):
            lib.msmd_gemm(*args)
        e1.record()
        e1.synchronize()
        t = e0.elapsed_time(e1)
        if t < best_t:
            best, best_t = v, t
    args[16] = act
    _TUNED[key] = best
    return best


def gemm(a, w, bias=None, residual=None, act=ACT_NONE, out=None, out_dtype=None, *, M=None, K=None, lda=None,
         rows_per_batch=0, a_batch_stride=0, batch=1, strideA=0, strideW=0, strideC=0, strideBias=0, strideR=0,
         N=None, ldw=None, ldc=None, z_out=None, p_drop=0.0, rng_state=None, site=0, variant=None, flags=None):
    _need_cuda(a, w, bias, residual)
    lib = _lib.load()
    if isinstance(w, Split) and not isinstance(a, Split):
        if not a.is_contiguous() or a.shape[-1] % 32:
            raise ValueError("split GEMM: pass a contiguous fp32 tensor with a last dim % 32 == 0, or a Split")
        a = to_split(a)
    if isinstance(a, Split) and not isinstance(w, Split):
        raise TypeError("split activations need split weights")
    if isinstance(a, Split) and out_dtype is None and out is None:
        out_dtype = torch.float32
    if K is None:
        K = a.shape[-1]
    if M is None:
        M = a.numel() // K
    if N is None:
        N = w.shape[-2]
    if lda is None:
        lda = K
    if ldw is None:
        ldw = w.shape[-1]
    out_dtype = out_dtype or a.dtype
    if out is None:
        lead = a.shape[:-1] if a.numel() // a.shape[-1] == M and batch == 1 else (M,)
        out = empty((*lead, N), a.device, out_dtype)
    if ldc is None:
        ldc = N
    ldr = residual.stride(-2) if residual is not None and residual.dim() >= 2 else N
    if bias is not None and bias.dtype != torch.float32:
        raise TypeError("bias must be fp32")
    trace = _trace_begin(M, N, K, batch, _dt(a))
    if variant is None:
        variant = _GEMM_DEFAULT["split_variant"] if isinstance(a, Split) else _GEMM_DEFAULT["variant"]
        if GEMM_ROUTER is not None and not isinstance(a, Split):
            variant = GEMM_ROUTER(M, N, K, batch) or variant
    flags = _GEMM_DEFAULT["flags"] if flags is None else flags
    if isinstance(w, Split) and w.below_32:
        flags |= GEMM_W_BELOW_32
    act = act | (variant << 8) | flags
    args = [_p(a), _p(w), _p(bias), _p(residual), _p(out), M, N, K, _dt(a), _dt(out), lda, rows_per_batch,
            a_batch_stride, ldw, ldc, ldr, act, batch, strideA, strideW, strideC, strideBias, strideR, _stream()]
    if (GEMM_AUTOTUNE and variant == 0 and a.dtype == torch.bfloat16 and K % 64 == 0
            and 2.0 * M * N * K * batch >= _TUNE_MIN_FLOP):
        key = (M, N, K, batch, out.dtype, act, bias is not None, residual is not None, rows_per_batch > 0, lda, ldc)
        v = _TUNED.get(key)
        if v is None:
            v = _autotune_gemm(lib, args, key, out, residual)
        args[16] = act | (v << 8)
    train = z_out is not None or p_drop > 0.0
    if train or trace is not None:
        ex = (*args[:-1], _p(z_out), float(p_drop), _p(rng_state), int(site), args[-1])
    if train:
        _lib.check(lib.msmd_gemm_ex(*ex), "msmd_gemm_ex")
    else:
        _lib.check(lib.msmd_gemm(*args), "msmd_gemm")
    _trace_end(trace, lib.msmd_gemm_route, ex if trace is not None else None)
    return out


GEMM_LN_TILE = None


def gemm_ln(a, w, bias=None, residual=None, act=ACT_NONE, out=None, out_dtype=None, *, a_stats=None, w_colsum=None,
            r_stats=None, r_gamma=None, r_beta=None, stats_out=False, eps=1e-5):
    _need_cuda(a, w, bias, residual)
    lib = _lib.load()
    K = a.shape[-1]
    M = a.numel() // K
    N = w.shape[0]
    out_dtype = out_dtype or a.dtype
    if out is None:
        out = empty((*a.shape[:-1], N), a.device, out_dtype)
    st, slab_out, slab_in = None, 0, 0
    if stats_out:
        slab_out = 64 if N % 128 == 0 else 32
        st = empty((N // slab_out, M, 2), a.device, torch.float32)
    sin = a_stats if a_stats is not None else r_stats
    if sin is not None:
        cols = K if a_stats is not None else N
        if sin.dim() != 3 or sin.shape[1] != M or sin.shape[2] != 2 or cols % sin.shape[0]:
            raise ValueError("gemm_ln: statistics must be (cols / slab, M, 2)")
        slab_in = cols // sin.shape[0]
    for t in (bias, w_colsum, r_gamma, r_beta, a_stats, r_stats):
        if t is not None and (t.dtype != torch.float32 or not t.is_contiguous()):
            raise TypeError("gemm_ln: bias / colsum / gamma / beta / stats must be contiguous fp32")
    ldr = residual.stride(-2) if residual is not None and residual.dim() >= 2 else N
    trace = _trace_begin(M, N, K, 1, _dt(a))
    hint = 66 if GEMM_LN_ALL_IN_ONE else ((GEMM_LN_ROUTER(M, N, K) or 0) if GEMM_LN_ROUTER is not None else (GEMM_LN_TILE or 0))
    args = (_p(a), _p(w), _p(bias), _p(residual), _p(out), M, N, K, _dt(a), _dt(out), a.stride(-2) if a.dim() >= 2 else K,
            w.stride(0), N, ldr, act | GEMM_LN_FLAGS | (hint << 8), _p(a_stats), _p(w_colsum), _p(r_stats), _p(r_gamma),
            _p(r_beta), _p(st), slab_in, slab_out, float(eps), _stream())
    _lib.check(lib.msmd_gemm_ln(*args), "msmd_gemm_ln")
    _trace_end(trace, lib.msmd_gemm_ln_route, args)
    return (out, st) if st is not None else out


def fold_layernorm(w, b, gamma, beta, dtype):
    w32, g32, be32 = w.float(), gamma.float(), beta.float()
    wf = (w32 * g32[None, :]).to(dtype).contiguous()
    cs = wf.float().sum(dim=1).contiguous()
    bf = (w32 @ be32 + (b.float() if b is not None else 0.0)).contiguous()
    return wf, cs, bf


def gemm_act_bwd(dy, wt, z, act, p_drop=0.0, rng_state=None, site=0):
    _need_cuda(dy, wt, z)
    K = dy.shape[-1]
    M = dy.numel() // K
    N = wt.shape[0]
    if z.numel() != M * N or not z.is_contiguous() or not dy.is_contiguous():
        raise ValueError("gemm_act_bwd: z must be the contiguous (M, N) pre-activation")
    out = torch.empty_like(z)
    trace = _trace_begin(M, N, K, 1, _dt(dy))
    _lib.check(_lib.load().msmd_gemm_actbwd(_p(dy), _p(wt), _p(z), _p(out), M, N, K, _dt(dy), _dt(out), K, wt.stride(0),
                                            act | (_GEMM_DEFAULT["flags"] & GEMM_PAIRED_STORES), float(p_drop), _p(rng_state),
                                            int(site), _stream()), "msmd_gemm_actbwd")
    _trace_end(trace)
    return out


def exp_set_tuning(key, value):
    raise _lib.MsmdLibraryError("msmd_exp_set_tuning: the experimental library and its tuning keys were removed; "
                                "use the per-call `variant` / `flags` / `splits` arguments")


g_tn_split = True


def gemm_tn(a, b, want_colsum=False, *, M=None, N=None, K=None, lda=None, ldb=None, batch=1, strideA=0, strideB=0,
            b_rows_per_window=0, b_window_stride=0, out=None, colsum_out=None, accumulate=False, splits=0):
    _need_cuda(a, b)
    if a.dtype != torch.bfloat16 or b.dtype != torch.bfloat16:
        raise TypeError("gemm_tn takes bf16 operands")
    lib = _lib.load()
    M = a.shape[-2] if M is None else M
    N = a.shape[-1] if N is None else N
    K = b.shape[-1] if K is None else K
    lda = a.stride(-2) if lda is None else lda
    ldb = b.stride(-2) if ldb is None else ldb
    if out is None:
        out = torch.empty((batch, N, K) if batch > 1 else (N, K), device=a.device, dtype=torch.float32)
    elif out.dtype != torch.float32 or not out.is_contiguous() or out.numel() != batch * N * K:
        raise ValueError("gemm_tn out must be a contiguous fp32 (N, K) tensor")
    cs = colsum_out if colsum_out is not None else (
        torch.empty(N, device=a.device, dtype=torch.float32) if want_colsum else None)
    nws = lib.msmd_gemm_tn_workspace(M, N, K, batch) if g_tn_split else 0
    ws = torch.empty(nws, device=a.device, dtype=torch.uint8) if nws > 0 else None
    _lib.check(lib.msmd_gemm_tn(_p(a), _p(b), _p(out), _p(cs), M, N, K, lda, ldb, K, batch, strideA, strideB, N * K,
                                b_rows_per_window, b_window_stride, int(bool(accumulate)) | (int(splits) << 8), _p(ws), nws,
                                _stream()), "msmd_gemm_tn")
    return (out, cs) if (want_colsum or colsum_out is not None) else out


def conv1d_cl(x, w_packed, bias=None, *, kernel, stride, act=ACT_NONE, out_dtype=None):
    B, T, C = x.shape
    T_out = (T - kernel) // stride + 1
    out = empty((B, T_out, w_packed.shape[0]), x.device, out_dtype or x.dtype)
    gemm(x, w_packed, bias, None, act, out=out, M=B * T_out, K=kernel * C, lda=stride * C, rows_per_batch=T_out,
         a_batch_stride=T * C)
    return out


def layernorm(x, gamma, beta, residual=None, post_add=None, act=ACT_NONE, eps=1e-5, out_dtype=None, post_act=ACT_NONE,
              split=None):
    _need_cuda(x, gamma, beta)
    lib = _lib.load()
    cols = x.shape[-1]
    rows = x.numel() // cols
    if split:
        if x.dtype != torch.float32 or (residual is not None and residual.dtype != torch.float32):
            raise TypeError("layernorm(split=...) takes fp32 input")
        y = torch.empty(x.shape, device=x.device, dtype=torch.float32) if split == "both" else None
        ys = empty(tuple(x.shape), x.device, SPLIT)
        _lib.check(lib.msmd_layernorm_f16x2(_p(x), _p(residual), _p(gamma), _p(beta), _p(post_add), _p(y), _p(ys), rows,
                                            cols, eps, act | (post_act << 8), _stream()), "msmd_layernorm_f16x2")
        return (y, ys) if split == "both" else ys
    y = torch.empty(x.shape, device=x.device, dtype=out_dtype or x.dtype)
    _lib.check(lib.msmd_layernorm(_p(x), _p(residual), _p(gamma), _p(beta), _p(post_add), _p(y), rows, cols, eps,
                                  act | (post_act << 8),
                                  _dt(x), _dt(y), _stream()), "msmd_layernorm")
    return y


def layernorm_pre(x, pre_gamma, pre_beta, residual, gamma, beta, eps=1e-5):
    _need_cuda(x, gamma, beta, pre_gamma, pre_beta)
    cols = x.shape[-1]
    rows = x.numel() // cols
    y = torch.empty_like(x)
    _lib.check(_lib.load().msmd_layernorm_pre(_p(x), _p(pre_gamma), _p(pre_beta), _p(residual), _p(gamma), _p(beta), _p(y),
                                              rows, cols, eps, _dt(x), _stream()), "msmd_layernorm_pre")
    return y


def dropout(x, p, rng_state, site, residual=None, out=None):
    _need_cuda(x, rng_state)
    x = x.contiguous()
    if residual is not None:
        residual = residual.contiguous()
    out = torch.empty_like(x) if out is None else out
    _lib.check(_lib.load().msmd_dropout(_p(x), _p(residual), _p(out), x.numel(), float(p), _p(rng_state), int(site),
                                        _dt(x), _stream()), "msmd_dropout")
    return out


def _prefetch_ranges(tensors):
    ts = []
    for t in tensors:
        t = t.t if isinstance(t, Split) else t
        if t is not None and t.is_cuda and t.is_contiguous():
            ts.append(t)
    ts = ts[:4]
    ptrs = (ctypes.c_void_p * 4)(*([t.data_ptr() for t in ts] + [None] * (4 - len(ts))))
    nbytes = (ctypes.c_long * 4)(*([t.numel() * t.element_size() for t in ts] + [0] * (4 - len(ts))))
    return ptrs, nbytes, len(ts)


def _attn_args(mask, scale, n_heads, q, k, v, *rest):
    B, Tq, _ = q.shape
    Tk = k.shape[1]
    if mask is not None:
        assert mask.dtype in (torch.bool, torch.uint8) and mask.shape == (Tq, Tk) and mask.is_contiguous()
    ts = (q, k, v) + rest
    return (*[_p(t) for t in ts], B, n_heads, Tq, Tk, *[t.stride(i) for t in ts for i in (0, 1)], float(scale), _p(mask))


def attention(q, k, v, n_heads, scale, mask=None, out=None, p_drop=0.0, rng_state=None, site=0, out_dtype=None,
              prefetch=None):
    _need_cuda(q, k, v)
    lib = _lib.load()
    B, Tq, d = q.shape
    assert d == n_heads * 64 and q.stride(-1) == 1 and k.stride(-1) == 1 and v.stride(-1) == 1
    split = isinstance(q, Split)
    if split and (not (isinstance(k, Split) and isinstance(v, Split)) or p_drop > 0.0):
        raise TypeError("split attention: q, k, v must all be Split (inference only)")
    if out is None:
        out = empty((B, Tq, d), q.device, out_dtype or SPLIT) if split else torch.empty(B, Tq, d, device=q.device, dtype=q.dtype)
    args = _attn_args(mask, scale, n_heads, q, k, v, out)
    drop = (float(p_drop), _p(rng_state), int(site)) if p_drop > 0.0 else ()
# ... 1040 lines not shown
```

Before: 812,600 frames/s.

## Split leftover GEMM tail tiles into half/quarter pieces to fill idle workgroups

```diff
diff --git a/include/msmd_hip.h b/include/msmd_hip.h
--- a/include/msmd_hip.h
+++ b/include/msmd_hip.h
@@ -26,6 +26,7 @@
 #define MSMD_GEMM_ONE_TILE_PER_WORKGROUP (1 << 19)
 #define MSMD_GEMM_NO_256_TILE (1 << 20)
 #define MSMD_GEMM_W_BELOW_32 (1 << 21)
+#define MSMD_GEMM_WHOLE_TILES (1 << 22)
 
 int msmd_spin_us(float us, long* ticks_out, msmd_stream_t stream);
 
@@ -53,6 +54,8 @@
                        int in_dtype, int out_dtype, long lda, long ldw, long ldc, long ldr, int act, const float* a_stats,
                        const float* w_colsum, const float* r_stats, const float* r_gamma, const float* r_beta,
                        float* stats_out, int slab_in, int slab_out, float eps, msmd_stream_t stream);
+
+int msmd_gemm8_plan(int M, int N, int workgroups, int act, int* items, int capacity);
 
 int msmd_gemm_actbwd(const void* A, const void* W, const void* Z, void* C, int M, int N, int K, int in_dtype, int out_dtype,
                      long lda, long ldw, int act, float p_drop, const unsigned long* rng_state, unsigned int site,
diff --git a/ubisoft-laforge-msmd_amd/csrc/gemm.hip b/ubisoft-laforge-msmd_amd/csrc/gemm.hip
--- a/ubisoft-laforge-msmd_amd/csrc/gemm.hip
+++ b/ubisoft-laforge-msmd_amd/csrc/gemm.hip
@@ -17,6 +17,7 @@
   const float* r_stats = nullptr; int r_nt = 0; const float* r_gamma = nullptr; const float* r_beta = nullptr;
   float* stats_out = nullptr; float ln_eps = 1e-5f;
   int stagger_ticks = 0;
+  int cut = 1;
 };
 
 enum : int {
@@ -24,14 +25,16 @@
   GF_ACT_BWD = 8,
   GF_ONE_TILE = 16, GF_NO_256 = 32,
   GF_W_BELOW_32 = 64,
+  GF_WHOLE_TILES = 128,
 };
 struct GemmActWord { int act, hint, flags; };
 static constexpr GemmActWord gemm_unpack_act(int act) {
-  return {act & 0xff, (act >> 8) & 0xff, ((act >> 16) & 7) | (((act >> 19) & 7) << 4)};
+  return {act & 0xff, (act >> 8) & 0xff, ((act >> 16) & 7) | (((act >> 19) & 15) << 4)};
 }
 static_assert(gemm_unpack_act(MSMD_GEMM_WRITE_THROUGH).flags == GF_WRITE_THROUGH && gemm_unpack_act(MSMD_GEMM_PAIRED_STORES).flags == GF_PAIRED_STORES &&
               gemm_unpack_act(MSMD_GEMM_STAGGER).flags == GF_STAGGER && gemm_unpack_act(MSMD_GEMM_ONE_TILE_PER_WORKGROUP).flags == GF_ONE_TILE &&
-              gemm_unpack_act(MSMD_GEMM_NO_256_TILE).flags == GF_NO_256 && gemm_unpack_act(MSMD_GEMM_W_BELOW_32).flags == GF_W_BELOW_32 && gemm_unpack_act(~0).flags == (0x7f & ~GF_ACT_BWD),
+              gemm_unpack_act(MSMD_GEMM_NO_256_TILE).flags == GF_NO_256 && gemm_unpack_act(MSMD_GEMM_W_BELOW_32).flags == GF_W_BELOW_32 && gemm_unpack_act(MSMD_GEMM_WHOLE_TILES).flags == GF_WHOLE_TILES &&
+              gemm_unpack_act(~0).flags == (0xff & ~GF_ACT_BWD),
               "internal flag bits follow include/msmd_hip.h; no bit of `act` sets the internal one");
 enum : int {
   GV_GENERIC = 0,
@@ -959,11 +962,31 @@
   else gemm_epilogue_split<FM, FN, ACTK>(p, acc0, z, m0 + wm, n0 + wn, fr, fq);
 }
 
+__host__ __device__ inline void gemm8_xcd_run(int n, int xcd, int& run0, int& run_n) {
+  run0 = xcd < (n & 7) ? xcd * ((n >> 3) + 1) : (n & 7) * ((n >> 3) + 1) + (xcd - (n & 7)) * (n >> 3);
+  run_n = (n >> 3) + (xcd < (n & 7) ? 1 : 0);
+}
+__host__ __device__ inline bool gemm8_piece(int M, int nt, int ntiles, int whole, int cut, int pid, int& m0, int& n0) {
+  if (cut <= 1) return false;
+  int run0, run_n;
+  gemm8_xcd_run((ntiles - whole) * cut, pid & 7, run0, run_n);
+  if ((pid >> 3) >= run_n) return false;
+  const int pi = run0 + (pid >> 3), tile = whole + pi / cut, sub = pi % cut;
+  const int m_tile = tile / nt, n_tile = tile - m_tile * nt;
+  m0 = m_tile * 256 + (cut == 2 ? sub : sub >> 1) * 128;
+  n0 = n_tile * 256 + (cut == 4 ? (sub & 1) * 128 : 0);
+  return m0 < M;
+}
+constexpr int GEMM8_RING = 2 * 4 * 128 * 128;
+constexpr int GEMM8_LDS_PIECES = GEMM8_RING + 2 * 128 * 128;
+template <int N> __device__ __forceinline__ void vm_wait() { asm volatile("s_waitcnt vmcnt(%0)" ::"n"(N) : "memory"); }
+
 template <typename TI, int EPIA, int SPLIT = 0>
 __global__ __launch_bounds__(512) __attribute__((amdgpu_waves_per_eu(2, 2))) void gemm8_kernel(const GemmArgs p) {
   typedef typename std::conditional<(SPLIT & 3) == 2, float, TI>::type TO;
   constexpr bool WS = (SPLIT & 4) != 0;
   constexpr int EPI = epia_family(EPIA), ACTK = epia_act(EPIA);
+  constexpr bool PIECES = EPI == 1;
   static_assert(SPLIT == 0 || (EPI == 1 && __is_same(TI, f16_t)), "split operands: fp16 planes, plain epilogue");
   constexpr int HALF = 128 * 128;
   constexpr int BUF = 4 * HALF;
@@ -971,8 +994,9 @@
 
   const int pid = blockIdx.x, ntiles = p.mt * p.nt, nwg = gridDim.x;
   const int xcd = pid & 7;
-  const int run0 = (xcd < (ntiles & 7) ? xcd * ((ntiles >> 3) + 1) : (ntiles & 7) * ((ntiles >> 3) + 1) + (xcd - (ntiles & 7)) * (ntiles >> 3));
-  const int run_n = (ntiles >> 3) + (xcd < (ntiles & 7) ? 1 : 0);
+  const int whole = PIECES && p.cut > 1 ? ntiles - ntiles % nwg : ntiles;
+  int run0, run_n;
+  gemm8_xcd_run(whole, xcd, run0, run_n);
   const int stride = (nwg >> 3) + (xcd < (nwg & 7) ? 1 : 0);
   int tl = pid >> 3;
   const bf16_t* __restrict__ A = (const bf16_t*)p.A;
@@ -983,29 +1007,35 @@
 
   unsigned src[4][2];
   int m0 = 0, n0 = 0;
+  int pm0 = 0, pn0 = 0;
+  auto set_src = [&]() {
+    int ln = lane;
+    asm volatile("" : "+v"(ln));
+#pragma unroll
+    for (int i = 0; i < 2; ++i) {
+      const int row = (i * 8 + wid) * 8 + (ln >> 3), phys = ln & 7;
+      const int c = phys ^ ((row >> 1) & 7);
+#pragma unroll
+      for (int h = 0; h < 2; ++h) {
+        src[h][i] = (unsigned)((a_row_offset(p, min(m0 + h * 128 + row, p.M - 1)) + c * 8) * 2);
+        src[2 + h][i] = (unsigned)(((long)min(n0 + h * 128 + row, p.N - 1) * p.ldw + c * 8) * 2);
+      }
+    }
+  };
   auto set_tile = [&](int t) {
     const int m_tile = (run0 + t) / p.nt, n_tile = (run0 + t) - m_tile * p.nt;
     m0 = m_tile * 256; n0 = n_tile * 256;
-    int ln = lane;
-    asm volatile("" : "+v"(ln));
-#pragma unroll
-    for (int i = 0; i < 2; ++i) {
-      const int row = (i * 8 + wid) * 8 + (ln >> 3), phys = ln & 7;
-      const int c = phys ^ ((row >> 1) & 7);
-#pragma unroll
-      for (int h = 0; h < 2; ++h) {
-        src[h][i] = (unsigned)((a_row_offset(p, min(m0 + h * 128 + row, p.M - 1)) + c * 8) * 2);
-        src[2 + h][i] = (unsigned)(((long)min(n0 + h * 128 + row, p.N - 1) * p.ldw + c * 8) * 2);
-      }
-    }
-  };
+    set_src();
+  };
+  auto set_piece = [&]() { m0 = pm0; n0 = pn0; set_src(); };
   const unsigned dma_base = wid * 1024;
-  auto stage = [&](int which, int kt, unsigned bufoff) {
+  auto stage_at = [&](int which, int kt, unsigned ldsoff) {
 #pragma unroll
     for (int i = 0; i < 2; ++i)
       __builtin_amdgcn_global_load_lds((gbl_void_t*)((const char*)(which < 2 ? A : W) + (size_t)(src[which][i] + (unsigned)kt * 128u)),
-                                       (lds_void_t*)(smem + (dma_base + bufoff + which * HALF + i * 8192)), 16, 0, 0);
-  };
+                                       (lds_void_t*)(smem + (dma_base + ldsoff + i * 8192)), 16, 0, 0);
+  };
+  auto stage = [&](int which, int kt, unsigned bufoff) { stage_at(which, kt, bufoff + which * HALF); };
 
   const int fr = lane & 15, fq = lane >> 4;
   const int sw = (fr >> 1) & 7;
@@ -1025,18 +1055,18 @@
     }
   };
 
-  auto read_x = [&](int h) {
+  auto read_x = [&](int h, unsigned off = 0) {
 #pragma unroll
     for (int j = 0; j < 4; ++j) {
-      fx[0][j] = *(const u32x4*)(smem + xa0 + h * HALF + j * 2048);
-      fx[1][j] = *(const u32x4*)(smem + xa1 + h * HALF + j * 2048);
-    }
-  };
-  auto read_w = [&](int g, u32x4 (&fw)[2][2]) {
+      fx[0][j] = *(const u32x4*)(smem + (xa0 + off) + h * HALF + j * 2048);
+      fx[1][j] = *(const u32x4*)(smem + (xa1 + off) + h * HALF + j * 2048);
+    }
+  };
+  auto read_w = [&](int g, u32x4 (&fw)[2][2], unsigned off = 0) {
 #pragma unroll
     for (int i = 0; i < 2; ++i) {
-      fw[0][i] = *(const u32x4*)(smem + wa0 + g * HALF + i * 2048);
-      fw[1][i] = *(const u32x4*)(smem + wa1 + g * HALF + i * 2048);
+      fw[0][i] = *(const u32x4*)(smem + (wa0 + off) + g * HALF + i * 2048);
+      fw[1][i] = *(const u32x4*)(smem + (wa1 + off) + g * HALF + i * 2048);
     }
   };
   auto quadrant = [&](f32x4 (&a)[2][4], const u32x4 (&fw)[2][2], const u32x4 (&fs)[2]) {
@@ -1132,6 +1162,258 @@
   stage(2, 1, BUF); stage(0, 1, BUF); stage(3, 1, BUF);
   asm volatile("s_waitcnt vmcnt(6)" ::: "memory");
   __builtin_amdgcn_s_barrier();
+
+  auto piece_loop = [&](auto CUT_) {
+    constexpr int CUT = decltype(CUT_)::value, NWH = CUT == 2 ? 2 : 1, NS = CUT == 2 ? 3 : 5;
+    constexpr int SB = (1 + NWH) * HALF, LP = 2 * (1 + NWH), LAST = (NS - 1) * SB;
+    static_assert(NS * SB <= GEMM8_LDS_PIECES && (NS - 2) * LP < 64, "ring fits the LDS, the counts fit vmcnt");
+    auto stage_k = [&](int kt, unsigned off) {
+      stage_at(2, kt, off + HALF); stage_at(0, kt, off);
+      if constexpr (NWH == 2) stage_at(3, kt, off + 2 * HALF);
+    };
+    auto reads = [&](unsigned off) {
+      read_w(0, fw0, off - HALF);
+      if constexpr (NWH == 2) read_w(1, fw1, off - HALF);
+      read_x(0, off);
+      asm volatile("s_waitcnt lgkmcnt(0)" ::: "memory");
+      if constexpr (WS) {
+        scale_w(fw0, fs0);
+        if constexpr (NWH == 2) scale_w(fw1, fs1);
+      }
+    };
+    auto mult = [&]() {
+      quadrant(acc[0][0], fw0, fs0);
+      if constexpr (NWH == 2) quadrant(acc[0][1], fw1, fs1);
+    };
+#pragma unroll
+    for (int s = 1; s < NS - 1; ++s) stage_k(min(s, nk - 1), s * SB);
+    vm_wait<(NS - 2) * LP>();
+    __builtin_amdgcn_s_barrier();
+    if (wr == 1) __builtin_amdgcn_s_barrier();
+    unsigned rd = 0, fill = LAST;
+    for (int t = 0; t + NS - 1 < nk; ++t) {
+      G8_BAR();
+      stage_k(t + NS - 1, fill);
+      fill = fill == LAST ? 0 : fill + SB;
+      reads(rd);
+      rd = rd == LAST ? 0 : rd + SB;
+      vm_wait<(NS - 2) * LP>();
+      G8_BAR();
+      mult();
+    }
+    auto tail = [&](auto U_) {
+      constexpr int U = decltype(U_)::value;
+      if (nk > U) {
+        G8_BAR();
+        reads(rd);
+        rd = rd == LAST ? 0 : rd + SB;
+        if constexpr (U > 0) vm_wait<(U - 1) * LP>();
+        G8_BAR();
+        mult();
+      }
+    };
+    if constexpr (NS == 5) { tail(std::integral_constant<int, 3>{}); tail(std::integral_constant<int, 2>{}); }
+    tail(std::integral_constant<int, 1>{});
+    tail(std::integral_constant<int, 0>{});
+    if (wr == 0) __builtin_amdgcn_s_barrier();
+  };
+
+  bool more = false, piece_next = false;
+  auto epilogue = [&](auto PC_) {
+    constexpr bool PC = decltype(PC_)::value;
+    const int em0 = m0, en0 = n0;
+    int el = lane;
+    asm volatile("" : "+v"(el));
+    const int efr = el & 15, efq = el >> 4;
+    const bool colok = !(PC && p.cut == 4) || el < 32;
+    const int ecl = colok ? el : el - 32;
+    const int ncol = en0 + ecl * 4;
+    f32x4 cbias = f32x4{0.f, 0.f, 0.f, 0.f}, cx = f32x4{1.f, 1.f, 1.f, 1.f}, cy = f32x4{0.f, 0.f, 0.f, 0.f};
+    if (p.bias) cbias = *(const f32x4*)(p.bias + ncol);
+    if constexpr (EPI == 2) cx = *(const f32x4*)(p.w_colsum + ncol);
+    if constexpr (EPI == 3) {
+      if (p.r_stats) { cx = *(const f32x4*)(p.r_gamma + ncol); cy = *(const f32x4*)(p.r_beta + ncol); }
+    }
+    float mu_l = 0.f, rs_l = 1.f;
+    if constexpr (EPI >= 2) {
+      if (ln_stats) {
+        const int r32 = el & 31;
+        const unsigned base = 2 * BUF + wid * 4096 + (((r32 >> 3) * 4 + ((r32 & 7) >> 1)) << 4) + ((r32 & 1) << 3);
+        float Sf[4], Qf[4];
+#pragma unroll
+        for (int f = 0; f < 4; ++f) {
+          f32x2 w[4];
+#pragma unroll
+          for (int q = 0; q < 4; ++q) {
+            const int t = f + 4 * q;
+            w[q] = *(const f32x2*)(smem + base + (t >> 2) * 1024 + ((t & 3) << 8));
+            if (t >= ln_nt) w[q] = f32x2{0.f, 0.f};
+          }
+          Sf[f] = (w[0][0] + w[1][0]) + (w[2][0] + w[3][0]);
+          Qf[f] = (w[0][1] + w[1][1]) + (w[2][1] + w[3][1]);
+        }
+        if (ln_nt > 16) {
+          const f32x2* rp = (const f32x2*)ln_stats + min(em0 + (r32 >> 3) * 64 + wid * 8 + (r32 & 7), p.M - 1);
+#pragma unroll
+          for (int f = 0; f < 4; ++f)
+            for (int t = 16 + f; t < ln_nt; t += 4) { const f32x2 w = rp[(long)t * p.M]; Sf[f] += w[0]; Qf[f] += w[1]; }
+        }
+        const float S = (Sf[0] + Sf[1]) + (Sf[2] + Sf[3]), Q = (Qf[0] + Qf[1]) + (Qf[2] + Qf[3]);
+        const float inv_cols = 1.0f / (float)(EPI == 2 ? p.K : p.N);
+        mu_l = S * inv_cols;
+        rs_l = rsqrtf(fmaxf(Q * inv_cols - mu_l * mu_l, 0.f) + p.ln_eps);
+        asm volatile("s_waitcnt lgkmcnt(0)" ::: "memory");
+      }
+    }
+    tl += stride;
+    more = !PC && tl < run_n;
+    piece_next = PIECES && !PC && !more && gemm8_piece(p.M, p.nt, ntiles, whole, p.cut, pid, pm0, pn0);
+    if (more) {
+      set_tile(tl);
+      stage(2, 0, 0); stage(0, 0, 0); stage(3, 0, 0); stage(1, 0, 0);
+      ln_request();
+    } else if (piece_next) {
+      set_piece();
+      stage_at(2, 0, HALF); stage_at(0, 0, 0);
+      if (p.cut == 2) stage_at(3, 0, 2 * HALF);
+    }
+    auto write_block = [&](const f32x4 (&q0)[2][4], const f32x4 (&q1)[2][4]) {
+#pragma unroll
+      for (int g = 0; g < 2; ++g)
+#pragma unroll
+        for (int i = 0; i < 2; ++i)
+#pragma unroll
+          for (int j = 0; j < 4; ++j) {
+            const int row = j * 16 + efr, c = g * 32 + wc * 8 + i * 4 + efq;
+            *(f32x4*)(smem + BUF + row * 1024 + ((c ^ efr) << 4)) = g == 0 ? q0[i][j] : q1[i][j];
+          }
+    };
+    auto finish_block = [&](int ps) {
+      if constexpr ((SPLIT & 3) == 2) {
+        f32x4 rr[8];
+        if (has_r) {
+#pragma unroll
+          for (int it = 0; it < 8; ++it) {
+            const int m = min(em0 + ps * 64 + wid * 8 + it, p.M - 1);
+            rr[it] = *(const f32x4*)((const float*)p.R + (long)m * p.ldr + ncol);
+          }
+        }
+#pragma unroll
+        for (int it = 0; it < 8; ++it) {
+          const int row = wid * 8 + it, m = em0 + ps * 64 + row;
+          const f32x4 a = *(const f32x4*)(smem + BUF + row * 1024 + ((el ^ (row & 15)) << 4));
+          f32x4 o;
+#pragma unroll
+          for (int e = 0; e < 4; ++e) {
+            o[e] = act_out_c<float, ACTK>(WS ? fmaf(a[e], MSMD_SPLIT_INV, cbias[e]) : a[e] + cbias[e], p.act);
+            if (has_r) o[e] += rr[it][e];
+          }
+          if (m < p.M && colok) {
+            if (wt) store16_wt((float*)p.C + (long)m * p.ldc + ncol, __builtin_bit_cast(u32x4, o));
+            else *(f32x4*)((float*)p.C + (long)m * p.ldc + ncol) = o;
+          }
+        }
+      } else if constexpr ((SPLIT & 3) == 1) {
+        const bool odd = el & 1;
+        const long coff = 2L * en0 + ((ecl >> 3) << 6) + (((ecl >> 1) & 3) << 3) + (odd ? 32 : 0);
+        auto swap1 = [](unsigned x) { return (unsigned)__builtin_amdgcn_mov_dpp((int)x, 0xB1, 0xF, 0xF, false); };
+        u32x4 rr[8];
+        if (has_r) {
+#pragma unroll
+          for (int it = 0; it < 8; ++it) {
+            const int m = min(em0 + ps * 64 + wid * 8 + it, p.M - 1);
+            rr[it] = *(const u32x4*)((const f16_t*)p.R + (long)m * 2 * p.ldr + coff);
+          }
+        }
+#pragma unroll
+        for (int it = 0; it < 8; ++it) {
+          const int row = wid * 8 + it, m = em0 + ps * 64 + row;
+          const f32x4 a = *(const f32x4*)(smem + BUF + row * 1024 + ((el ^ (row & 15)) << 4));
+          float v[4];
+#pragma unroll
+          for (int e = 0; e < 4; ++e) v[e] = act_split<ACTK>(WS ? fmaf(a[e], MSMD_SPLIT_INV, cbias[e]) : a[e] + cbias[e], p.act);
+          if (has_r) {
+            const unsigned g0 = swap1(odd ? rr[it][0] : rr[it][2]), g1 = swap1(odd ? rr[it][1] : rr[it][3]);
+            const f16x2 h01 = __builtin_bit_cast(f16x2, odd ? g0 : rr[it][0]), h23 = __builtin_bit_cast(f16x2, odd ? g1 : rr[it][1]);
+            const f16x2 l01 = __builtin_bit_cast(f16x2, odd ? rr[it][2] : g0), l23 = __builtin_bit_cast(f16x2, odd ? rr[it][3] : g1);
+            v[0] += unsplit_f16x2(h01[0], l01[0]); v[1] += unsplit_f16x2(h01[1], l01[1]);
+            v[2] += unsplit_f16x2(h23[0], l23[0]); v[3] += unsplit_f16x2(h23[1], l23[1]);
+          }
+          f16_t h[4], l[4];
+#pragma unroll
+          for (int e = 0; e < 4; ++e) split_f16x2(v[e], h[e], l[e]);
+          const unsigned hp0 = __builtin_bit_cast(unsigned, f16x2{h[0], h[1]}), hp1 = __builtin_bit_cast(unsigned, f16x2{h[2], h[3]});
+          const unsigned lp0 = __builtin_bit_cast(unsigned, f16x2{l[0], l[1]}), lp1 = __builtin_bit_cast(unsigned, f16x2{l[2], l[3]});
+          const unsigned g0 = swap1(odd ? hp0 : lp0), g1 = swap1(odd ? hp1 : lp1);
+          const u32x4 o = odd ? u32x4{g0, g1, lp0, lp1} : u32x4{hp0, hp1, g0, g1};
+          if (m < p.M && colok) {
+            if (wt) store16_wt((f16_t*)p.C + (long)m * 2 * p.ldc + coff, o);
+            else *(u32x4*)((f16_t*)p.C + (long)m * 2 * p.ldc + coff) = o;
+          }
+        }
+      } else {
+      V4 rr[8];
+      if (EPI != 2 && has_r) {
+#pragma unroll
+        for (int it = 0; it < 8; ++it) {
+          const int m = min(em0 + ps * 64 + wid * 8 + it, p.M - 1);
+          rr[it] = *(const V4*)((const TO*)p.R + (long)m * p.ldr + ncol);
+        }
+      }
+#pragma unroll
+      for (int it = 0; it < 8; ++it) {
+        const int row = wid * 8 + it, m = em0 + ps * 64 + row;
+        const f32x4 a = *(const f32x4*)(smem + BUF + row * 1024 + ((el ^ (row & 15)) << 4));
+        float mu = 0.f, rs = 1.f;
+        if constexpr (EPI >= 2) {
+          mu = __int_as_float(__builtin_amdgcn_readlane(__float_as_int(mu_l), ps * 8 + it));
+          rs = __int_as_float(__builtin_amdgcn_readlane(__float_as_int(rs_l), ps * 8 + it));
+        }
+        float v[4];
+#pragma unroll
+        for (int e = 0; e < 4; ++e) {
+          float x = a[e];
+          if constexpr (EPI == 2) x = rs * (x - mu * cx[e]);
+          v[e] = act_out_c<TO, ACTK>(x + cbias[e], p.act);
+          if constexpr (EPI == 3) v[e] += fmaf(((float)rr[it][e] - mu) * rs, cx[e], cy[e]);
+          else if (has_r) v[e] += (float)rr[it][e];
+        }
+        const V4 o = pack4<TO>(v[0], v[1], v[2], v[3]);
+        if (m < p.M && colok) {
+          if (wt) store8_wt((TO*)p.C + (long)m * p.ldc + ncol, __builtin_bit_cast(u32x2, o));
+          else *(V4*)((TO*)p.C + (long)m * p.ldc + ncol) = o;
+        }
+        if constexpr (EPI == 3) {
+          if (p.stats_out) {
+            float S = 0.f, Q = 0.f;
+#pragma unroll
+            for (int e = 0; e < 4; ++e) { const float w = (float)o[e]; S += w; Q = fmaf(w, w, Q); }
+#pragma unroll
+            for (int d : {4, 8, 1, 2}) { S += __shfl_xor(S, d, 64); Q += __shfl_xor(Q, d, 64); }
+            if ((el & 15) == 0 && m < p.M) *(f32x2*)(p.stats_out + ((long)((en0 >> 6) + (el >> 4)) * p.M + m) * 2) = f32x2{S, Q};
+          }
+        }
+      }
+      }
+    };
+    if (wr == 0) write_block(acc[0][0], acc[0][1]);
+    G8_EBAR();
+    finish_block(0);
+    G8_EBAR();
+    if (wr == 1) write_block(acc[0][0], acc[0][1]);
+    G8_EBAR();
+    finish_block(1);
+    if constexpr (!PC) {
+    G8_EBAR();
+    if (wr == 0) write_block(acc[1][0], acc[1][1]);
+    G8_EBAR();
+    finish_block(2);
+    G8_EBAR();
+    if (wr == 1) write_block(acc[1][0], acc[1][1]);
+    G8_EBAR();
+    finish_block(3);
+    }
+  };
 
   while (true) {
     if (wr == 1) __builtin_amdgcn_s_barrier();
@@ -1182,196 +1464,28 @@
     ktile(nk - 1, std::integral_constant<int, 2>{});
     if (wr == 0) __builtin_amdgcn_s_barrier();
     if (nk & 1) { xa0 ^= BUF; xa1 ^= BUF; wa0 ^= BUF; wa1 ^= BUF; }
-
-    const int em0 = m0, en0 = n0;
-    int el = lane;
-    asm volatile("" : "+v"(el));
-    const int efr = el & 15, efq = el >> 4;
-    const int ncol = en0 + el * 4;
-    f32x4 cbias = f32x4{0.f, 0.f, 0.f, 0.f}, cx = f32x4{1.f, 1.f, 1.f, 1.f}, cy = f32x4{0.f, 0.f, 0.f, 0.f};
-    if (p.bias) cbias = *(const f32x4*)(p.bias + ncol);
-    if constexpr (EPI == 2) cx = *(const f32x4*)(p.w_colsum + ncol);
-    if constexpr (EPI == 3) {
-      if (p.r_stats) { cx = *(const f32x4*)(p.r_gamma + ncol); cy = *(const f32x4*)(p.r_beta + ncol); }
-    }
-    float mu_l = 0.f, rs_l = 1.f;
-    if constexpr (EPI >= 2) {
-      if (ln_stats) {
-        const int r32 = el & 31;
-        const unsigned base = 2 * BUF + wid * 4096 + (((r32 >> 3) * 4 + ((r32 & 7) >> 1)) << 4) + ((r32 & 1) << 3);
-        float Sf[4], Qf[4];
-#pragma unroll
-        for (int f = 0; f < 4; ++f) {
-          f32x2 w[4];
-#pragma unroll
-          for (int q = 0; q < 4; ++q) {
-            const int t = f + 4 * q;
-            w[q] = *(const f32x2*)(smem + base + (t >> 2) * 1024 + ((t & 3) << 8));
-            if (t >= ln_nt) w[q] = f32x2{0.f, 0.f};
-          }
-          Sf[f] = (w[0][0] + w[1][0]) + (w[2][0] + w[3][0]);
-          Qf[f] = (w[0][1] + w[1][1]) + (w[2][1] + w[3][1]);
-        }
-        if (ln_nt > 16) {
-          const f32x2* rp = (const f32x2*)ln_stats + min(em0 + (r32 >> 3) * 64 + wid * 8 + (r32 & 7), p.M - 1);
-#pragma unroll
-          for (int f = 0; f < 4; ++f)
-            for (int t = 16 + f; t < ln_nt; t += 4) { const f32x2 w = rp[(long)t * p.M]; Sf[f] += w[0]; Qf[f] += w[1]; }
-        }
-        const float S = (Sf[0] + Sf[1]) + (Sf[2] + Sf[3]), Q = (Qf[0] + Qf[1]) + (Qf[2] + Qf[3]);
-        const float inv_cols = 1.0f / (float)(EPI == 2 ? p.K : p.N);
-        mu_l = S * inv_cols;
-        rs_l = rsqrtf(fmaxf(Q * inv_cols - mu_l * mu_l, 0.f) + p.ln_eps);
-        asm volatile("s_waitcnt lgkmcnt(0)" ::: "memory");
-      }
-    }
-    tl += stride;
-    const bool more = tl < run_n;
-    if (more) {
-      set_tile(tl);
-      stage(2, 0, 0); stage(0, 0, 0); stage(3, 0, 0); stage(1, 0, 0);
-      ln_request();
-    }
-    auto write_block = [&](const f32x4 (&q0)[2][4], const f32x4 (&q1)[2][4]) {
-#pragma unroll
-      for (int g = 0; g < 2; ++g)
-#pragma unroll
-        for (int i = 0; i < 2; ++i)
-#pragma unroll
-          for (int j = 0; j < 4; ++j) {
-            const int row = j * 16 + efr, c = g * 32 + wc * 8 + i * 4 + efq;
-            *(f32x4*)(smem + BUF + row * 1024 + ((c ^ efr) << 4)) = g == 0 ? q0[i][j] : q1[i][j];
-          }
-    };
-    auto finish_block = [&](int ps) {
-      if constexpr ((SPLIT & 3) == 2) {
-        f32x4 rr[8];
-        if (has_r) {
-#pragma unroll
-          for (int it = 0; it < 8; ++it) {
-            const int m = min(em0 + ps * 64 + wid * 8 + it, p.M - 1);
-            rr[it] = *(const f32x4*)((const float*)p.R + (long)m * p.ldr + ncol);
-          }
-        }
-#pragma unroll
-        for (int it = 0; it < 8; ++it) {
-          const int row = wid * 8 + it, m = em0 + ps * 64 + row;
-          const f32x4 a = *(const f32x4*)(smem + BUF + row * 1024 + ((el ^ (row & 15)) << 4));
-          f32x4 o;
-#pragma unroll
-          for (int e = 0; e < 4; ++e) {
-            o[e] = act_out_c<float, ACTK>(WS ? fmaf(a[e], MSMD_SPLIT_INV, cbias[e]) : a[e] + cbias[e], p.act);
-            if (has_r) o[e] += rr[it][e];
-          }
-          if (m < p.M) {
-            if (wt) store16_wt((float*)p.C + (long)m * p.ldc + ncol, __builtin_bit_cast(u32x4, o));
-            else *(f32x4*)((float*)p.C + (long)m * p.ldc + ncol) = o;
-          }
-        }
-      } else if constexpr ((SPLIT & 3) == 1) {
-        const bool odd = el & 1;
-        const long coff = 2L * en0 + ((el >> 3) << 6) + (((el >> 1) & 3) << 3) + (odd ? 32 : 0);
-        auto swap1 = [](unsigned x) { return (unsigned)__builtin_amdgcn_mov_dpp((int)x, 0xB1, 0xF, 0xF, false); };
-        u32x4 rr[8];
-        if (has_r) {
-#pragma unroll
-          for (int it = 0; it < 8; ++it) {
-            const int m = min(em0 + ps * 64 + wid * 8 + it, p.M - 1);
-            rr[it] = *(const u32x4*)((const f16_t*)p.R + (long)m * 2 * p.ldr + coff);
-          }
-        }
-#pragma unroll
-        for (int it = 0; it < 8; ++it) {
-          const int row = wid * 8 + it, m = em0 + ps * 64 + row;
-          const f32x4 a = *(const f32x4*)(smem + BUF + row * 1024 + ((el ^ (row & 15)) << 4));
-          float v[4];
-#pragma unroll
-          for (int e = 0; e < 4; ++e) v[e] = act_split<ACTK>(WS ? fmaf(a[e], MSMD_SPLIT_INV, cbias[e]) : a[e] + cbias[e], p.act);
-          if (has_r) {
-            const unsigned g0 = swap1(odd ? rr[it][0] : rr[it][2]), g1 = swap1(odd ? rr[it][1] : rr[it][3]);
-            const f16x2 h01 = __builtin_bit_cast(f16x2, odd ? g0 : rr[it][0]), h23 = __builtin_bit_cast(f16x2, odd ? g1 : rr[it][1]);
-            const f16x2 l01 = __builtin_bit_cast(f16x2, odd ? rr[it][2] : g0), l23 = __builtin_bit_cast(f16x2, odd ? rr[it][3] : g1);
-            v[0] += unsplit_f16x2(h01[0], l01[0]); v[1] += unsplit_f16x2(h01[1], l01[1]);
-            v[2] += unsplit_f16x2(h23[0], l23[0]); v[3] += unsplit_f16x2(h23[1], l23[1]);
-          }
-          f16_t h[4], l[4];
-#pragma unroll
-          for (int e = 0; e < 4; ++e) split_f16x2(v[e], h[e], l[e]);
-          const unsigned hp0 = __builtin_bit_cast(unsigned, f16x2{h[0], h[1]}), hp1 = __builtin_bit_cast(unsigned, f16x2{h[2], h[3]});
-          const unsigned lp0 = __builtin_bit_cast(unsigned, f16x2{l[0], l[1]}), lp1 = __builtin_bit_cast(unsigned, f16x2{l[2], l[3]});
-          const unsigned g0 = swap1(odd ? hp0 : lp0), g1 = swap1(odd ? hp1 : lp1);
-          const u32x4 o = odd ? u32x4{g0, g1, lp0, lp1} : u32x4{hp0, hp1, g0, g1};
-          if (m < p.M) {
-            if (wt) store16_wt((f16_t*)p.C + (long)m * 2 * p.ldc + coff, o);
-            else *(u32x4*)((f16_t*)p.C + (long)m * 2 * p.ldc + coff) = o;
-          }
-        }
-      } else {
-      V4 rr[8];
-      if (EPI != 2 && has_r) {
-#pragma unroll
-        for (int it = 0; it < 8; ++it) {
-          const int m = min(em0 + ps * 64 + wid * 8 + it, p.M - 1);
-          rr[it] = *(const V4*)((const TO*)p.R + (long)m * p.ldr + ncol);
-        }
-      }
-#pragma unroll
-      for (int it = 0; it < 8; ++it) {
-        const int row = wid * 8 + it, m = em0 + ps * 64 + row;
-        const f32x4 a = *(const f32x4*)(smem + BUF + row * 1024 + ((el ^ (row & 15)) << 4));
-        float mu = 0.f, rs = 1.f;
-        if constexpr (EPI >= 2) {
-          mu = __int_as_float(__builtin_amdgcn_readlane(__float_as_int(mu_l), ps * 8 + it));
-          rs = __int_as_float(__builtin_amdgcn_readlane(__float_as_int(rs_l), ps * 8 + it));
-        }
-        float v[4];
-#pragma unroll
-        for (int e = 0; e < 4; ++e) {
-          float x = a[e];
-          if constexpr (EPI == 2) x = rs * (x - mu * cx[e]);
-          v[e] = act_out_c<TO, ACTK>(x + cbias[e], p.act);
-          if constexpr (EPI == 3) v[e] += fmaf(((float)rr[it][e] - mu) * rs, cx[e], cy[e]);
-          else if (has_r) v[e] += (float)rr[it][e];
-        }
-        const V4 o = pack4<TO>(v[0], v[1], v[2], v[3]);
-        if (m < p.M) {
-          if (wt) store8_wt((TO*)p.C + (long)m * p.ldc + ncol, __builtin_bit_cast(u32x2, o));
-          else *(V4*)((TO*)p.C + (long)m * p.ldc + ncol) = o;
-        }
-        if constexpr (EPI == 3) {
-          if (p.stats_out) {
-            float S = 0.f, Q = 0.f;
-#pragma unroll
-            for (int e = 0; e < 4; ++e) { const float w = (float)o[e]; S += w; Q = fmaf(w, w, Q); }
-#pragma unroll
-            for (int d : {4, 8, 1, 2}) { S += __shfl_xor(S, d, 64); Q += __shfl_xor(Q, d, 64); }
-            if ((el & 15) == 0 && m < p.M) *(f32x2*)(p.stats_out + ((long)((en0 >> 6) + (el >> 4)) * p.M + m) * 2) = f32x2{S, Q};
-          }
-        }
-      }
-      }
-    };
-    if (wr == 0) write_block(acc[0][0], acc[0][1]);
-    G8_EBAR();
-    finish_block(0);
-    G8_EBAR();
-    if (wr == 1) write_block(acc[0][0], acc[0][1]);
-    G8_EBAR();
-    finish_block(1);
-    G8_EBAR();
-    if (wr == 0) write_block(acc[1][0], acc[1][1]);
-    G8_EBAR();
-    finish_block(2);
-    G8_EBAR();
-    if (wr == 1) write_block(acc[1][0], acc[1][1]);
-    G8_EBAR();
-    finish_block(3);
+    epilogue(std::false_type{});
     if (!more) break;
     G8_EBAR();
     set_tile(tl);
     stage(2, 1, BUF); stage(0, 1, BUF); stage(3, 1, BUF);
     asm volatile("s_waitcnt vmcnt(6)" ::: "memory");
     __builtin_amdgcn_s_barrier();
+  }
+  if constexpr (PIECES) {
+    if (piece_next) {
+      G8_EBAR();
+      set_piece();
+#pragma unroll
+      for (int g = 0; g < 2; ++g)
+#pragma unroll
+        for (int i = 0; i < 2; ++i)
+#pragma unroll
+          for (int j = 0; j < 4; ++j) acc[0][g][i][j] = f32x4{0.f, 0.f, 0.f, 0.f};
+      if (p.cut == 2) piece_loop(std::integral_constant<int, 2>{});
+      else piece_loop(std::integral_constant<int, 4>{});
+      epilogue(std::true_type{});
+    }
   }
 #undef G8_BAR
 #undef G8_EBAR
@@ -1481,11 +1595,25 @@
   return fill >= 0.75 && (K >= 1024 || fill >= 0.878);
 }
 
-constexpr int GEMM8_RING = 2 * 4 * 128 * 128;
-template <auto KFN, int LDS>
+constexpr double GEMM8_PIECE_FIXED = 0.3;
+static int gemm8_cut(int tiles, int G) {
+  if (G <= 0 || (G & 7) || tiles <= G) return 1;
+  const int r = tiles % G;
+  if (r == 0) return 1;
+  int best = 1;
+  double best_t = 1.0;
+  for (int s = 2; s <= 4; s *= 2) {
+    const double t = 1.0 / s + GEMM8_PIECE_FIXED;
+    if (r * s <= G && t < best_t) { best = s; best_t = t; }
+  }
+  return best;
+}
+
+template <auto KFN, int LDS, bool PIECES = false>
 static int launch_gemm8(GemmArgs& p, hipStream_t st) {
   p.mt = (p.M + 255) / 256; p.nt = p.N / 256;
   const int tiles = p.mt * p.nt, cap = gemm8_workgroup_cap();
+  p.cut = PIECES && !(p.flags & GF_WHOLE_TILES) ? gemm8_cut(tiles, cap) : 1;
   if (tiles <= 512) p.flags |= GF_WRITE_THROUGH;
   return gemm_launch_kernel<KFN>(dim3(tiles < cap ? tiles : cap), 512, LDS, st, p);
 }
@@ -1528,7 +1656,7 @@
       if (!gemm8s_takes(p, batch, sizeof(TO) == 2)) return -1;
       return dispatch_code<11, 21>(epia(EPI_PLAIN, p.act), [&](auto c) {
         return dispatch_code<0, 1>((p.flags & GF_W_BELOW_32) != 0, [&](auto ws) {
-          return launch_gemm8<gemm8_kernel<f16_t, decltype(c)::value, (sizeof(TO) == 4 ? 2 : 1) + 4 * decltype(ws)::value>, GEMM8_RING>(p, st);
+          return launch_gemm8<gemm8_kernel<f16_t, decltype(c)::value, (sizeof(TO) == 4 ? 2 : 1) + 4 * decltype(ws)::value>, GEMM8_LDS_PIECES, true>(p, st);
         });
       });
     default: return -1;
@@ -1570,7 +1698,8 @@
       if (!gemm8_takes(p, batch, 2)) return -1;
       return dispatch_code<11, 21, 12, 22, 13>(gemm_epia(p, true), [&](auto c) {
         constexpr int E = decltype(c)::value;
-        return launch_gemm8<gemm8_kernel<TI, E>, GEMM8_RING + (epia_family(E) >= EPI_LN_OPERAND ? 8 * 4096 : 0)>(p, st);
+        constexpr bool LN = epia_family(E) >= EPI_LN_OPERAND;
+        return launch_gemm8<gemm8_kernel<TI, E>, LN ? GEMM8_RING + 8 * 4096 : GEMM8_LDS_PIECES, !LN>(p, st);
       });
     }
   }
@@ -1657,7 +1786,7 @@
       if ((c.N & 3) || c.ldc % 32 || c.strideC % 32 || c.strideC2 % 32 || (c.residual && (c.ldr % 32 || c.strideR % 32))) return -1;
       if (c.bias && (((uintptr_t)c.bias & 15) || (c.strideBias & 3))) return -1;
     }
-    p = gemm_args(c, u.act, flags & (GF_WRITE_THROUGH | GF_W_BELOW_32), c.out_dtype == MSMD_F32 ? 4 : 0, 2);
+    p = gemm_args(c, u.act, flags & (GF_WRITE_THROUGH | GF_W_BELOW_32 | GF_WHOLE_TILES), c.out_dtype == MSMD_F32 ? 4 : 0, 2);
     return gemm_split_route(p, nz, c.out_dtype == MSMD_F16X2, u.hint, flags);
   }
   if (c.in_dtype == MSMD_F32 ? (c.out_dtype != MSMD_F32 && c.out_dtype != MSMD_F16 && c.out_dtype != MSMD_BF16)
@@ -1732,6 +1861,26 @@
   GemmArgs p;
   return gemm_plan(p, gemm_ex_call(A, W, bias, residual, C, M, N, K, in_dtype, out_dtype, lda, rows_per_batch, a_batch_stride, ldw, ldc, ldr,
                                    act, batch, strideA, strideW, strideC, strideBias, strideR, z_out, p_drop, rng_state, site));
+}
+
+extern "C" int msmd_gemm8_plan(int M, int N, int workgroups, int act, int* items, int capacity) {
+  if (M <= 0 || N <= 0 || (N % 256) || workgroups <= 0) return -1;
+  const int mt = (M + 255) / 256, nt = N / 256, ntiles = mt * nt, nwg = ntiles < workgroups ? ntiles : workgroups;
+  const int cut = (gemm_unpack_act(act).flags & GF_WHOLE_TILES) ? 1 : gemm8_cut(ntiles, workgroups);
+  const int whole = cut > 1 ? ntiles - ntiles % nwg : ntiles;
+  int n = 0;
+  auto put = [&](int pid, int m0, int n0, int rows, int cols) {
+    if (items && n < capacity) { int* it = items + 5L * n; it[0] = pid; it[1] = m0; it[2] = n0; it[3] = rows; it[4] = cols; }
+    ++n;
+  };
+  for (int pid = 0; pid < nwg; ++pid) {
+    int run0, run_n, m0, n0;
+    gemm8_xcd_run(whole, pid & 7, run0, run_n);
+    const int stride = (nwg >> 3) + ((pid & 7) < (nwg & 7) ? 1 : 0);
+    for (int tl = pid >> 3; tl < run_n; tl += stride) put(pid, (run0 + tl) / nt * 256, (run0 + tl) % nt * 256, 256, 256);
+    if (gemm8_piece(M, nt, ntiles, whole, cut, pid, m0, n0)) put(pid, m0, n0, 128, cut == 2 ? 256 : 128);
+  }
+  return n;
 }
 
 static int gemm_ln_plan(GemmArgs& p, const GemmCall& c) {
diff --git a/ubisoft-laforge-msmd_amd/ops.py b/ubisoft-laforge-msmd_amd/ops.py
--- a/ubisoft-laforge-msmd_amd/ops.py
+++ b/ubisoft-laforge-msmd_amd/ops.py
@@ -155,6 +155,7 @@
 GEMM_ONE_TILE_PER_WORKGROUP = 1 << 19
 GEMM_NO_256_TILE = 1 << 20
 GEMM_W_BELOW_32 = 1 << 21
+GEMM_WHOLE_TILES = 1 << 22
 GEMM_LN_FLAGS = 0
 GEMM_LN_ROUTER = None
 GEMM_LN_ALL_IN_ONE = False
@@ -181,6 +182,10 @@
 if os.environ.get("MSMD_GEMM_ONE_TILE", "0") == "1":
     _GEMM_DEFAULT["flags"] |= GEMM_ONE_TILE_PER_WORKGROUP
     GEMM_LN_FLAGS = GEMM_ONE_TILE_PER_WORKGROUP
+
+
+if os.environ.get("MSMD_GEMM_WHOLE_TILES", "0") == "1":
+    _GEMM_DEFAULT["flags"] |= GEMM_WHOLE_TILES
 
 
 if os.environ.get("MSMD_GEMM_NO_256", "0") == "1":
```

Result: no change. 815,300 frames/s (median of 4 runs) (+0.3%).
